# 0xPARC/plonky2-aes

Hardware: AMD Instinct MI355X
Metric: proofs/sec (AES-GCM 1 KiB circuit) (higher is better)
Workload: dtype u64 (Goldilocks field)

## Files before the change

bindings/plonky2-hip/src/ffi.rs:

```rust
#![allow(non_camel_case_types, dead_code)]
use std::os::raw::{c_char, c_int, c_long, c_void};

#[repr(C)] pub struct P2Builder { _private: [u8; 0] }
#[repr(C)] pub struct P2Circuit { _private: [u8; 0] }
#[repr(C)] pub struct P2Assignment { pub targets: *const u64, pub values: *const u64, pub count: usize }
#[repr(C)] #[derive(Default, Clone, Copy)]
pub struct P2CircuitInfo {
    pub degree_bits: u32, pub num_wires: u32, pub num_routed_wires: u32, pub num_constants_cols: u32, pub num_zs_cols: u32,
    pub num_quotient_cols: u32, pub num_luts: u32, pub num_ops: u32, pub num_levels: u32, pub num_slots: u32,
    pub num_virtual_targets: u32, pub num_fri_rounds: u32, pub proof_bytes: u64, pub zero_knowledge: u32, pub num_gate_kinds: u32,
    pub num_public_inputs: u32, pub hasher: u32,
}
#[repr(C)] pub struct P2KernelTime { pub name: [c_char; 48], pub ms: f32, pub count: u32 }
#[repr(C)] #[derive(Default, Clone, Copy, Debug)]
pub struct P2WitnessFault { pub kind: i32, pub op_kind: i32, pub input_index: i64, pub target: u64, pub gate_row: u32, pub computed: u64, pub found: u64 }

pub const P2_OK: c_int = 0;
pub const P2_PROOF_OK: c_int = 0;
pub const P2_VALUE_UNSET: u64 = u64::MAX;
pub const P2_FAULT_KINDS: [&str; 6] = ["NONE", "INPUT_NOT_CANONICAL", "INPUT_CONFLICT", "LOOKUP_MISS", "GENERATOR_CONFLICT", "NOT_SET"];
pub const P2_HASHER_POSEIDON: c_int = 0;
pub const P2_HASHER_KECCAK: c_int = 1;
pub const P2_POINT_WORDS: usize = 10;
pub const P2_SCALAR_LIMBS: usize = 5;
pub const P2_SCALAR_BITS: usize = 320;

#[link(name = "p2aes")]
extern "C" {
    pub fn p2_last_error() -> *const c_char;
    pub fn p2_builder_new() -> *mut P2Builder;
    pub fn p2_builder_new_zk() -> *mut P2Builder;
    pub fn p2_builder_new_config(zero_knowledge: c_int, hasher: c_int) -> *mut P2Builder;
    pub fn p2_builder_set_hasher(a0: *mut P2Builder, hasher: c_int) -> c_int;
    pub fn p2_builder_free(a0: *mut P2Builder);
    pub fn p2_builder_add_virtual_target(a0: *mut P2Builder) -> u64;
    pub fn p2_builder_constant(a0: *mut P2Builder, c: u64) -> u64;
    pub fn p2_builder_zero(a0: *mut P2Builder) -> u64;
    pub fn p2_builder_one(a0: *mut P2Builder) -> u64;
    pub fn p2_builder_arithmetic(a0: *mut P2Builder, c0: u64, c1: u64, m0: u64, m1: u64, addend: u64) -> u64;
    pub fn p2_builder_mul_const_add(a0: *mut P2Builder, c: u64, x: u64, y: u64) -> u64;
    pub fn p2_builder_add(a0: *mut P2Builder, x: u64, y: u64) -> u64;
    pub fn p2_builder_sub(a0: *mut P2Builder, x: u64, y: u64) -> u64;
    pub fn p2_builder_mul(a0: *mut P2Builder, x: u64, y: u64) -> u64;
    pub fn p2_builder_select(a0: *mut P2Builder, b: u64, x: u64, y: u64) -> u64;
    pub fn p2_builder_is_equal(a0: *mut P2Builder, x: u64, y: u64) -> u64;
    pub fn p2_builder_connect(a0: *mut P2Builder, x: u64, y: u64);
    pub fn p2_builder_register_public_input(a0: *mut P2Builder, t: u64) -> c_int;
    pub fn p2_builder_add_lookup_table_from_pairs(a0: *mut P2Builder, pairs: *const u16, n_pairs: usize) -> usize;
    pub fn p2_builder_add_lookup_from_index(a0: *mut P2Builder, looking_in: u64, lut_index: usize) -> u64;
    pub fn p2_builder_num_gates(a0: *const P2Builder) -> usize;
    pub fn p2_builder_build(a0: *mut P2Builder, blob: *mut *mut u8, blob_len: *mut usize) -> c_int;
    pub fn p2_blob_free(blob: *mut u8);
    pub fn p2_aes_sbox_lut(a0: *mut P2Builder) -> usize;
    pub fn p2_aes_byte_xor_lut(a0: *mut P2Builder) -> usize;
    pub fn p2_aes_gf_2_8_mul_lut(a0: *mut P2Builder) -> usize;
    pub fn p2_gcm_u8_unit_right_shift_lut(a0: *mut P2Builder) -> usize;
    pub fn p2_gcm_u8_bitref_lut(a0: *mut P2Builder) -> usize;
    pub fn p2_aes_add_virtual_byte_target(a0: *mut P2Builder, u8_table_idx: usize) -> u64;
    pub fn p2_aes_add_virtual_byte_target_unsafe(a0: *mut P2Builder) -> u64;
    pub fn p2_aes_state_sub_bytes(a0: *mut P2Builder, sbox_lut: usize, s: *const u64, out: *mut u64);
    pub fn p2_aes_state_mix_columns(a0: *mut P2Builder, xor_lut: usize, mul_lut: usize, s: *const u64, out: *mut u64);
    pub fn p2_aes_gf_2_8_mul(a0: *mut P2Builder, mul_lut: usize, x: u64, y: u64) -> u64;
    pub fn p2_aes_gf_2_8_add(a0: *mut P2Builder, xor_lut: usize, x: u64, y: u64) -> u64;
    pub fn p2_aes_key_expansion(a0: *mut P2Builder, nk: c_int, nr: c_int, xor_lut: usize, sbox_lut: usize, key: *const u64, out: *mut u64);
    pub fn p2_aes_encrypt_block(a0: *mut P2Builder, nr: c_int, xor_lut: usize, mul_lut: usize, sbox_lut: usize, state: *const u64, expanded_key: *const u64, out_state: *mut u64);
    pub fn p2_gcm_gctr(a0: *mut P2Builder, nr: c_int, xor_lut: usize, mul_lut: usize, sbox_lut: usize, expanded_key: *const u64, icb: *const u64, x: *const u64, len: usize, y: *mut u64);
    pub fn p2_gcm_right_shift_one(a0: *mut P2Builder, shift_lut: usize, v: *const u64, out: *mut u64);
    pub fn p2_gcm_inc32(a0: *mut P2Builder, block: *const u64, out: *mut u64);
    pub fn p2_gcm_gf_2_128_mul(a0: *mut P2Builder, xor_lut: usize, shift_lut: usize, bitref_lut: usize, x: *const u64, y: *const u64, out: *mut u64);
    pub fn p2_gcm_ghash(a0: *mut P2Builder, xor_lut: usize, shift_lut: usize, bitref_lut: usize, h: *const u64, x: *const u64, len: usize, out: *mut u64) -> c_int;
    pub fn p2_aes_gcm_build(a0: *mut P2Builder, nk: c_int, nr: c_int, L: usize, with_tag: c_int, key: *mut u64, nonce: *mut u64, pt: *mut u64, ct: *mut u64, tag: *mut u64) -> c_int;
    pub fn p2_builder_hash_n_to_m_no_pad(a0: *mut P2Builder, inputs: *const u64, n: usize, outputs: *mut u64, m: usize) -> c_int;
    pub fn p2_poseidon_cipher_build(a0: *mut P2Builder, L: usize, ks: *mut u64, m: *mut u64, nonce: *mut u64, ct: *mut u64) -> c_int;
    pub fn p2_native_hash_n_to_m_no_pad(in: *const u64, n: usize, out: *mut u64, m: usize);
    pub fn p2_native_poseidon_encrypt(ks10: *const u64, msg: *const u64, n_msg: usize, nonce2: *const u64, ct: *mut u64);
    pub fn p2_native_poseidon_decrypt(ks10: *const u64, ct: *const u64, n_ct: usize, nonce2: *const u64, l: usize, msg: *mut u64) -> c_int;
    pub fn p2_ecgfp5_group_order(out: *mut u64);
    pub fn p2_ecgfp5_generator(out: *mut u64);
    pub fn p2_ecgfp5_mul(k: *const u64, p: *const u64, out: *mut u64);
    pub fn p2_ecgfp5_add(p: *const u64, q: *const u64, out: *mut u64);
    pub fn p2_ecgfp5_neg(p: *const u64, out: *mut u64);
    pub fn p2_ecgfp5_is_in_subgroup(p: *const u64) -> c_int;
    pub fn p2_ecgfp5_compress(p: *const u64, w: *mut u64);
    pub fn p2_ecgfp5_decompress(w: *const u64, out: *mut u64) -> c_int;
    pub fn p2_ecgfp5_random_scalar(out: *mut u64) -> c_int;
    pub fn p2_ecgfp5_random_point(out: *mut u64) -> c_int;
    pub fn p2_ecgfp5_encode_binary(limbs: *const u32, out: *mut u64) -> c_int;
    pub fn p2_ecgfp5_random_scalar_seeded(seed: u64, out: *mut u64);
    pub fn p2_ecgfp5_random_point_seeded(seed: u64, out: *mut u64);
    pub fn p2_ecgfp5_encode_binary_seeded(limbs: *const u32, seed: u64, out: *mut u64);
    pub fn p2_ecgfp5_decode_binary(p: *const u64, limbs: *mut u32);
    pub fn p2_elgamal_encrypt(pk: *const u64, nonce: *const u64, msg: *const u64, c0: *mut u64, c1: *mut u64) -> c_int;
    pub fn p2_elgamal_decrypt(sk: *const u64, c0: *const u64, c1: *const u64, msg: *mut u64) -> c_int;
    pub fn p2_hashed_elgamal_encrypt(pk: *const u64, nonce: *const u64, msg: *const u64, c0: *mut u64, ct: *mut u64) -> c_int;
    pub fn p2_hashed_elgamal_decrypt(sk: *const u64, c0: *const u64, ct: *const u64, msg: *mut u64) -> c_int;
    pub fn p2_builder_add_virtual_point_target(a0: *mut P2Builder, out: *mut u64);
    pub fn p2_builder_constant_point(a0: *mut P2Builder, p: *const u64, out: *mut u64);
    pub fn p2_builder_add_virtual_biguint320_target(a0: *mut P2Builder, bits: *mut u64);
    pub fn p2_builder_multiply_point(a0: *mut P2Builder, bits: *const u64, p: *const u64, out: *mut u64) -> c_int;
    pub fn p2_builder_add_point(a0: *mut P2Builder, p: *const u64, q: *const u64, out: *mut u64);
    pub fn p2_builder_public_key(a0: *mut P2Builder, sk_bits: *const u64, pk: *mut u64) -> c_int;
    pub fn p2_builder_elgamal_encrypt(a0: *mut P2Builder, pk: *const u64, nonce_bits: *const u64, msg: *const u64, c0: *mut u64, c1: *mut u64) -> c_int;
    pub fn p2_builder_hashed_elgamal_encrypt(a0: *mut P2Builder, pk: *const u64, nonce_bits: *const u64, msg: *const u64, c0: *mut u64, ct: *mut u64) -> c_int;
    pub fn p2_selftest_host(seed: u64, n_reductions: usize, n_permutations: usize) -> c_int;
    pub fn p2_selftest_device(seed: u64, threads: usize, device: c_int) -> c_int;
    pub fn p2_host_poseidon_known(states: *mut u64, n_perm: usize, kind: c_int, rows: u32, parts: c_int) -> c_int;
    pub fn p2_host_partial_rounds(states: *mut u64, count: usize) -> c_int;
    pub fn p2_host_hash_leaves(data: *const u64, cols: usize, active_cols: usize, num_leaves: usize, digests: *mut u64) -> c_int;
    pub fn p2_native_gf_2_8_mul(a: u8, b: u8) -> u8;
    pub fn p2_native_aes_key_expansion(key: *const u8, nk: c_int, nr: c_int, out: *mut u8);
    pub fn p2_native_aes_encrypt_block(key: *const u8, nk: c_int, nr: c_int, in16: *const u8, out16: *mut u8);
    pub fn p2_native_gf_2_128_mul(x16: *const u8, y16: *const u8, out16: *mut u8);
    pub fn p2_native_ghash(h16: *const u8, x: *const u8, len: usize, out16: *mut u8);
    pub fn p2_native_gctr(key: *const u8, nk: c_int, nr: c_int, icb16: *const u8, x: *const u8, len: usize, y: *mut u8);
    pub fn p2_native_aes_gcm_encrypt(key: *const u8, nk: c_int, nr: c_int, nonce12: *const u8, pt: *const u8, len: usize, ct: *mut u8, tag16: *mut u8);
    pub fn p2_native_keccak_hash_no_pad(in: *const u64, n: usize, out4: *mut u64);
    pub fn p2_native_keccak_two_to_one(l4: *const u64, r4: *const u64, out4: *mut u64);
    pub fn p2_native_keccak256(data: *const u8, len: usize, out32: *mut u8);
    pub fn p2_blob_info(blob: *const u8, len: usize, out: *mut P2CircuitInfo) -> c_int;
    pub fn p2_witness_schedule_check(blob: *const u8, len: usize, fuse: u32, out: *mut u32) -> c_int;
    pub fn p2_verify(blob: *const u8, blob_len: usize, verifier_data: *const u64, verifier_data_len: usize, proof: *const u8, proof_len: usize) -> c_int;
    pub fn p2_proof_compress(blob: *const u8, blob_len: usize, verifier_data: *const u64, verifier_data_len: usize, proof: *const u8, proof_len: usize, out: *mut u8, cap: usize, n_written: *mut usize) -> c_int;
    pub fn p2_proof_decompress(blob: *const u8, blob_len: usize, verifier_data: *const u64, verifier_data_len: usize, cproof: *const u8, cproof_len: usize, out: *mut u8, cap: usize, n_written: *mut usize) -> c_int;
    pub fn p2_verify_compressed(blob: *const u8, blob_len: usize, verifier_data: *const u64, verifier_data_len: usize, cproof: *const u8, cproof_len: usize) -> c_int;
    pub fn p2_proof_public_inputs(blob: *const u8, blob_len: usize, proof: *const u8, proof_len: usize, out: *mut u64, cap: usize, n_written: *mut usize) -> c_int;
    pub fn p2_circuit_load(blob: *const u8, len: usize, device: c_int) -> *mut P2Circuit;
    pub fn p2_circuit_free(a0: *mut P2Circuit);
    pub fn p2_circuit_verifier_data(a0: *const P2Circuit, out: *mut u64, cap: usize, n_written: *mut usize) -> c_int;
    pub fn p2_circuit_chunk_proofs(a0: *mut P2Circuit) -> usize;
    pub fn p2_circuit_set_zk_key(a0: *mut P2Circuit, key: *const u64) -> c_int;
    pub fn p2_circuit_set_zk_seed(a0: *mut P2Circuit, seed: u64) -> c_int;
    pub fn p2_circuit_proof_bytes(a0: *const P2Circuit) -> usize;
    pub fn p2_circuit_num_public_inputs(a0: *const P2Circuit) -> usize;
    pub fn p2_circuit_public_inputs(a0: *const P2Circuit, proof: *const u8, proof_len: usize, out: *mut u64, cap: usize, n_written: *mut usize) -> c_int;
    pub fn p2_prove_batch(a0: *mut P2Circuit, batch: usize, inputs: *const P2Assignment, proofs: *mut u8, status: *mut c_int) -> c_int;
    pub fn p2_prove_batch_multi(handles: *const *mut P2Circuit, n_handles: usize, batch: usize, inputs: *const P2Assignment, proofs: *mut u8, status: *mut c_int) -> c_int;
    pub fn p2_prove_batch_device(a0: *mut P2Circuit, batch: usize, targets: *const u64, n_targets: usize, d_values: *const u64, d_proofs: *mut u8, d_status: *mut c_int, stream: *mut c_void) -> c_int;
    pub fn p2_circuit_synchronize(a0: *mut P2Circuit) -> c_int;
    pub fn p2_prove_batch_outputs_device(a0: *mut P2Circuit, batch: usize, targets: *const u64, n_targets: usize, d_values: *const u64, out_targets: *const u64, n_out: usize, d_out: *mut u64, d_proofs: *mut u8, d_status: *mut c_int, stream: *mut c_void) -> c_int;
    pub fn p2_prove_batch_outputs(a0: *mut P2Circuit, batch: usize, inputs: *const P2Assignment, out_targets: *const u64, n_out: usize, out_values: *mut u64, proofs: *mut u8, status: *mut c_int) -> c_int;
    pub fn p2_witness_batch_device(a0: *mut P2Circuit, batch: usize, targets: *const u64, n_targets: usize, d_values: *const u64, out_targets: *const u64, n_out: usize, d_out: *mut u64, d_status: *mut c_int, stream: *mut c_void) -> c_int;
    pub fn p2_witness_batch(a0: *mut P2Circuit, batch: usize, inputs: *const P2Assignment, out_targets: *const u64, n_out: usize, out_values: *mut u64, status: *mut c_int) -> c_int;
    pub fn p2_witness_explain(a0: *mut P2Circuit, input: *const P2Assignment, status: *mut c_int, out: *mut c_void) -> c_int;
    pub fn p2_host_witness(blob: *const u8, len: usize, input: *const P2Assignment, out_targets: *const u64, n_out: usize, out_values: *mut u64, status: *mut c_int, fault: *mut c_void) -> c_int;
    pub fn p2_verify_batch(a0: *mut P2Circuit, batch: usize, proofs: *const u8, verifier_data: *const u64, vd_len: usize, status: *mut c_int) -> c_int;
    pub fn p2_verify_batch_device(a0: *mut P2Circuit, batch: usize, d_proofs: *const u8, verifier_data: *const u64, vd_len: usize, d_status: *mut c_int, stream: *mut c_void) -> c_int;
    pub fn p2_compress_batch(a0: *mut P2Circuit, batch: usize, proofs: *const u8, verifier_data: *const u64, vd_len: usize, out: *mut u8, lengths: *mut u32, status: *mut c_int) -> c_int;
    pub fn p2_decompress_batch(a0: *mut P2Circuit, batch: usize, cproofs: *const u8, lengths: *const u32, verifier_data: *const u64, vd_len: usize, out: *mut u8, status: *mut c_int) -> c_int;
    pub fn p2_verify_compressed_batch(a0: *mut P2Circuit, batch: usize, cproofs: *const u8, lengths: *const u32, verifier_data: *const u64, vd_len: usize, status: *mut c_int) -> c_int;
    pub fn p2_compress_batch_device(a0: *mut P2Circuit, batch: usize, d_proofs: *const u8, verifier_data: *const u64, vd_len: usize, d_out: *mut u8, d_lengths: *mut u32, d_status: *mut c_int, stream: *mut c_void) -> c_int;
    pub fn p2_decompress_batch_device(a0: *mut P2Circuit, batch: usize, d_cproofs: *const u8, d_lengths: *const u32, verifier_data: *const u64, vd_len: usize, d_out: *mut u8, d_status: *mut c_int, stream: *mut c_void) -> c_int;
    pub fn p2_verify_compressed_batch_device(a0: *mut P2Circuit, batch: usize, d_cproofs: *const u8, d_lengths: *const u32, verifier_data: *const u64, vd_len: usize, d_status: *mut c_int, stream: *mut c_void) -> c_int;
    pub fn p2_circuit_set_option(a0: *mut P2Circuit, name: *const c_char, value: c_long) -> c_int;
    pub fn p2_circuit_set_timing(a0: *mut P2Circuit, enable: c_int) -> c_int;
    pub fn p2_circuit_get_timing(a0: *mut P2Circuit, out: *mut P2KernelTime, cap: usize) -> usize;
    pub fn p2_gpu_device_count() -> c_int;
    pub fn p2_gpu_poseidon(states: *mut u64, n_perm: usize, device: c_int) -> c_int;
    pub fn p2_gpu_lde(coeffs: *const u64, cols: usize, degree_bits: c_int, rate_bits: c_int, lde: *mut u64, device: c_int) -> c_int;
    pub fn p2_gpu_intt(values: *const u64, cols: usize, degree_bits: c_int, coeffs: *mut u64, device: c_int) -> c_int;
    pub fn p2_gpu_merkle_cap(cols_major: *const u64, cols: usize, num_leaves: usize, cap_height: c_int, cap: *mut u64, device: c_int) -> c_int;
    pub fn p2_gpu_merkle_cap_hasher(cols_major: *const u64, cols: usize, num_leaves: usize, cap_height: c_int, hasher: c_int, cap: *mut u64, device: c_int) -> c_int;
    pub fn p2_gpu_hash_leaves(data: *const u64, cols: usize, active_cols: usize, num_leaves: usize, batch: usize, digests: *mut u64, device: c_int) -> c_int;
    pub fn p2_gpu_partial_rounds(states: *mut u64, count: usize, device: c_int) -> c_int;
    pub fn p2_gpu_merkle_level(child: *const u64, num_parents: usize, batch: usize, parent: *mut u64, device: c_int) -> c_int;
    pub fn p2_gpu_hash_fri_leaves(vals: *const u64, len: usize, arity: c_int, batch: usize, digests: *mut u64, device: c_int) -> c_int;
    pub fn p2_circuit_debug_read(a0: *mut P2Circuit, name: *const c_char, index: usize, out: *mut u64, cap: usize, n_written: *mut usize) -> c_int;
}
```

include/p2aes.h:

```cpp
#ifndef P2AES_H
#define P2AES_H
#include <stddef.h>
#include <stdint.h>

#ifdef __cplusplus
extern "C" {
#endif

enum {
    P2_OK = 0,
    P2_ERR_INVALID = 1,
    P2_ERR_NO_DEVICE = 2,
    P2_ERR_HIP = 3,
    P2_ERR_VERIFY = 4
};
enum {
    P2_PROOF_OK = 0,
    P2_PROOF_WITNESS_CONFLICT = 1,
    P2_PROOF_MISSING_INPUT = 2,
    P2_PROOF_ZETA_IN_SUBGROUP = 3,
    P2_PROOF_POW_NOT_FOUND = 4
};
enum {
    P2_VERIFY_OK = 0,
// ... 26 lines not shown
p2_target p2_builder_arithmetic(p2_builder*, uint64_t c0, uint64_t c1, p2_target m0, p2_target m1, p2_target addend);
p2_target p2_builder_mul_const_add(p2_builder*, uint64_t c, p2_target x, p2_target y);
p2_target p2_builder_add(p2_builder*, p2_target x, p2_target y);
p2_target p2_builder_sub(p2_builder*, p2_target x, p2_target y);
p2_target p2_builder_mul(p2_builder*, p2_target x, p2_target y);
p2_target p2_builder_select(p2_builder*, p2_target b, p2_target x, p2_target y);
p2_target p2_builder_is_equal(p2_builder*, p2_target x, p2_target y);
void p2_builder_connect(p2_builder*, p2_target x, p2_target y);
int p2_builder_register_public_input(p2_builder*, p2_target t);
size_t p2_builder_add_lookup_table_from_pairs(p2_builder*, const uint16_t* pairs, size_t n_pairs);
p2_target p2_builder_add_lookup_from_index(p2_builder*, p2_target looking_in, size_t lut_index);
size_t p2_builder_num_gates(const p2_builder*);
int p2_builder_build(p2_builder*, uint8_t** blob, size_t* blob_len);
void p2_blob_free(uint8_t* blob);

size_t p2_aes_sbox_lut(p2_builder*);
size_t p2_aes_byte_xor_lut(p2_builder*);
size_t p2_aes_gf_2_8_mul_lut(p2_builder*);
size_t p2_gcm_u8_unit_right_shift_lut(p2_builder*);
size_t p2_gcm_u8_bitref_lut(p2_builder*);
p2_target p2_aes_add_virtual_byte_target(p2_builder*, size_t u8_table_idx);
p2_target p2_aes_add_virtual_byte_target_unsafe(p2_builder*);
void p2_aes_state_sub_bytes(p2_builder*, size_t sbox_lut, const p2_target* s, p2_target* out);
void p2_aes_state_mix_columns(p2_builder*, size_t xor_lut, size_t mul_lut, const p2_target* s, p2_target* out);
p2_target p2_aes_gf_2_8_mul(p2_builder*, size_t mul_lut, p2_target x, p2_target y);
p2_target p2_aes_gf_2_8_add(p2_builder*, size_t xor_lut, p2_target x, p2_target y);
void p2_aes_key_expansion(p2_builder*, int nk, int nr, size_t xor_lut, size_t sbox_lut, const p2_target* key, p2_target* out);
void p2_aes_encrypt_block(p2_builder*, int nr, size_t xor_lut, size_t mul_lut, size_t sbox_lut, const p2_target* state,
                          const p2_target* expanded_key, p2_target* out_state);
void p2_gcm_gctr(p2_builder*, int nr, size_t xor_lut, size_t mul_lut, size_t sbox_lut, const p2_target* expanded_key,
                 const p2_target* icb, const p2_target* x, size_t len, p2_target* y);
void p2_gcm_right_shift_one(p2_builder*, size_t shift_lut, const p2_target* v, p2_target* out);
void p2_gcm_inc32(p2_builder*, const p2_target* block, p2_target* out);
void p2_gcm_gf_2_128_mul(p2_builder*, size_t xor_lut, size_t shift_lut, size_t bitref_lut, const p2_target* x,
                         const p2_target* y, p2_target* out);
int p2_gcm_ghash(p2_builder*, size_t xor_lut, size_t shift_lut, size_t bitref_lut, const p2_target* h, const p2_target* x,
                 size_t len, p2_target* out);
int p2_aes_gcm_build(p2_builder*, int nk, int nr, size_t L, int with_tag, p2_target* key, p2_target* nonce, p2_target* pt,
                     p2_target* ct, p2_target* tag);

int p2_builder_hash_n_to_m_no_pad(p2_builder*, const p2_target* inputs, size_t n, p2_target* outputs, size_t m);
int p2_poseidon_cipher_build(p2_builder*, size_t L, p2_target* ks, p2_target* m, p2_target* nonce, p2_target* ct);
void p2_native_hash_n_to_m_no_pad(const uint64_t* in, size_t n, uint64_t* out, size_t m);
void p2_native_poseidon_encrypt(const uint64_t* ks10, const uint64_t* msg, size_t n_msg, const uint64_t* nonce2, uint64_t* ct);
int p2_native_poseidon_decrypt(const uint64_t* ks10, const uint64_t* ct, size_t n_ct, const uint64_t* nonce2, size_t l, uint64_t* msg);

#define P2_POINT_WORDS 10
#define P2_SCALAR_LIMBS 5
#define P2_SCALAR_BITS 320
void p2_ecgfp5_group_order(uint64_t out[5]);
void p2_ecgfp5_generator(uint64_t out[10]);
void p2_ecgfp5_mul(const uint64_t k[5], const uint64_t p[10], uint64_t out[10]);
void p2_ecgfp5_add(const uint64_t p[10], const uint64_t q[10], uint64_t out[10]);
void p2_ecgfp5_neg(const uint64_t p[10], uint64_t out[10]);
int p2_ecgfp5_is_in_subgroup(const uint64_t p[10]);
void p2_ecgfp5_compress(const uint64_t p[10], uint64_t w[5]);
int p2_ecgfp5_decompress(const uint64_t w[5], uint64_t out[10]);
int p2_ecgfp5_random_scalar(uint64_t out[5]);
int p2_ecgfp5_random_point(uint64_t out[10]);
int p2_ecgfp5_encode_binary(const uint32_t limbs[5], uint64_t out[10]);
void p2_ecgfp5_random_scalar_seeded(uint64_t seed, uint64_t out[5]);
void p2_ecgfp5_random_point_seeded(uint64_t seed, uint64_t out[10]);
void p2_ecgfp5_encode_binary_seeded(const uint32_t limbs[5], uint64_t seed, uint64_t out[10]);
void p2_ecgfp5_decode_binary(const uint64_t p[10], uint32_t limbs[5]);
int p2_elgamal_encrypt(const uint64_t pk[10], const uint64_t nonce[5], const uint64_t msg[10], uint64_t c0[10], uint64_t c1[10]);
int p2_elgamal_decrypt(const uint64_t sk[5], const uint64_t c0[10], const uint64_t c1[10], uint64_t msg[10]);
int p2_hashed_elgamal_encrypt(const uint64_t pk[10], const uint64_t nonce[5], const uint64_t msg[5], uint64_t c0[10], uint64_t ct[5]);
int p2_hashed_elgamal_decrypt(const uint64_t sk[5], const uint64_t c0[10], const uint64_t ct[5], uint64_t msg[5]);
void p2_builder_add_virtual_point_target(p2_builder*, p2_target out[10]);
void p2_builder_constant_point(p2_builder*, const uint64_t p[10], p2_target out[10]);
void p2_builder_add_virtual_biguint320_target(p2_builder*, p2_target bits[320]);
int p2_builder_multiply_point(p2_builder*, const p2_target bits[320], const p2_target p[10], p2_target out[10]);
void p2_builder_add_point(p2_builder*, const p2_target p[10], const p2_target q[10], p2_target out[10]);
int p2_builder_public_key(p2_builder*, const p2_target sk_bits[320], p2_target pk[10]);
int p2_builder_elgamal_encrypt(p2_builder*, const p2_target pk[10], const p2_target nonce_bits[320], const p2_target msg[10],
                               p2_target c0[10], p2_target c1[10]);
int p2_builder_hashed_elgamal_encrypt(p2_builder*, const p2_target pk[10], const p2_target nonce_bits[320], const p2_target msg[5],
                                      p2_target c0[10], p2_target ct[5]);

int p2_selftest_host(uint64_t seed, size_t n_reductions, size_t n_permutations);
int p2_selftest_device(uint64_t seed, size_t threads, int device);
int p2_host_poseidon_known(uint64_t* states, size_t n_perm, int kind, uint32_t rows, int parts);
int p2_host_partial_rounds(uint64_t* states, size_t count);
int p2_host_hash_leaves(const uint64_t* data, size_t cols, size_t active_cols, size_t num_leaves, uint64_t* digests);

uint8_t p2_native_gf_2_8_mul(uint8_t a, uint8_t b);
void p2_native_aes_key_expansion(const uint8_t* key, int nk, int nr, uint8_t* out );
void p2_native_aes_encrypt_block(const uint8_t* key, int nk, int nr, const uint8_t* in16, uint8_t* out16);
void p2_native_gf_2_128_mul(const uint8_t* x16, const uint8_t* y16, uint8_t* out16);
void p2_native_ghash(const uint8_t* h16, const uint8_t* x, size_t len, uint8_t* out16);
void p2_native_gctr(const uint8_t* key, int nk, int nr, const uint8_t* icb16, const uint8_t* x, size_t len, uint8_t* y);
void p2_native_aes_gcm_encrypt(const uint8_t* key, int nk, int nr, const uint8_t* nonce12, const uint8_t* pt, size_t len,
                               uint8_t* ct, uint8_t* tag16);

void p2_native_keccak_hash_no_pad(const uint64_t* in, size_t n, uint64_t out4[4]);
void p2_native_keccak_two_to_one(const uint64_t l4[4], const uint64_t r4[4], uint64_t out4[4]);
void p2_native_keccak256(const uint8_t* data, size_t len, uint8_t out32[32]);

typedef struct {
    uint32_t degree_bits, num_wires, num_routed_wires, num_constants_cols, num_zs_cols, num_quotient_cols, num_luts,
        num_ops, num_levels, num_slots, num_virtual_targets, num_fri_rounds;
    uint64_t proof_bytes;
    uint32_t zero_knowledge, num_gate_kinds;
    uint32_t num_public_inputs;
    uint32_t hasher;
} p2_circuit_info;
int p2_blob_info(const uint8_t* blob, size_t len, p2_circuit_info* out);
int p2_witness_schedule_check(const uint8_t* blob, size_t len, uint32_t fuse, uint32_t out[4]);
int p2_verify(const uint8_t* blob, size_t blob_len, const uint64_t* verifier_data, size_t verifier_data_len,
              const uint8_t* proof, size_t proof_len);
int p2_proof_compress(const uint8_t* blob, size_t blob_len, const uint64_t* verifier_data, size_t verifier_data_len, const uint8_t* proof,
                      size_t proof_len, uint8_t* out, size_t cap, size_t* n_written);
int p2_proof_decompress(const uint8_t* blob, size_t blob_len, const uint64_t* verifier_data, size_t verifier_data_len, const uint8_t* cproof,
                        size_t cproof_len, uint8_t* out, size_t cap, size_t* n_written);
int p2_verify_compressed(const uint8_t* blob, size_t blob_len, const uint64_t* verifier_data, size_t verifier_data_len,
                         const uint8_t* cproof, size_t cproof_len);
int p2_proof_public_inputs(const uint8_t* blob, size_t blob_len, const uint8_t* proof, size_t proof_len, uint64_t* out, size_t cap,
                           size_t* n_written);

typedef struct p2_circuit p2_circuit;
p2_circuit* p2_circuit_load(const uint8_t* blob, size_t len, int device);
void p2_circuit_free(p2_circuit*);
int p2_circuit_verifier_data(const p2_circuit*, uint64_t* out, size_t cap, size_t* n_written);
size_t p2_circuit_chunk_proofs(p2_circuit*);
int p2_circuit_set_zk_key(p2_circuit*, const uint64_t key[4]);
int p2_circuit_set_zk_seed(p2_circuit*, uint64_t seed);
size_t p2_circuit_proof_bytes(const p2_circuit*);
size_t p2_circuit_num_public_inputs(const p2_circuit*);
int p2_circuit_public_inputs(const p2_circuit*, const uint8_t* proof, size_t proof_len, uint64_t* out, size_t cap, size_t* n_written);
typedef struct {
    const p2_target* targets;
    const uint64_t* values;
    size_t count;
} p2_assignment;
int p2_prove_batch(p2_circuit*, size_t batch, const p2_assignment* inputs, uint8_t* proofs, int* status);
int p2_prove_batch_multi(p2_circuit* const* handles, size_t n_handles, size_t batch, const p2_assignment* inputs,
                         uint8_t* proofs, int* status);
int p2_prove_batch_device(p2_circuit*, size_t batch, const p2_target* targets, size_t n_targets, const uint64_t* d_values,
                          uint8_t* d_proofs, int* d_status, void* stream);
int p2_circuit_synchronize(p2_circuit*);

#define P2_VALUE_UNSET UINT64_MAX
int p2_prove_batch_outputs_device(p2_circuit*, size_t batch, const p2_target* targets, size_t n_targets, const uint64_t* d_values,
                                  const p2_target* out_targets, size_t n_out, uint64_t* d_out, uint8_t* d_proofs, int* d_status, void* stream);
int p2_prove_batch_outputs(p2_circuit*, size_t batch, const p2_assignment* inputs, const p2_target* out_targets, size_t n_out,
                           uint64_t* out_values, uint8_t* proofs, int* status);
int p2_witness_batch_device(p2_circuit*, size_t batch, const p2_target* targets, size_t n_targets, const uint64_t* d_values,
                            const p2_target* out_targets, size_t n_out, uint64_t* d_out, int* d_status, void* stream);
int p2_witness_batch(p2_circuit*, size_t batch, const p2_assignment* inputs, const p2_target* out_targets, size_t n_out,
                     uint64_t* out_values, int* status);
typedef struct {
    int32_t kind;
    int32_t op_kind;
    int64_t input_index;
    p2_target target;
    uint32_t gate_row;
    uint64_t computed, found;
} p2_witness_fault;
enum {
    P2_FAULT_NONE = 0,
    P2_FAULT_INPUT_NOT_CANONICAL = 1,
    P2_FAULT_INPUT_CONFLICT = 2,
    P2_FAULT_LOOKUP_MISS = 3,
    P2_FAULT_GENERATOR_CONFLICT = 4,
    P2_FAULT_NOT_SET = 5
};
int p2_witness_explain(p2_circuit*, const p2_assignment* input, int* status, void* out);
int p2_host_witness(const uint8_t* blob, size_t len, const p2_assignment* input, const p2_target* out_targets, size_t n_out,
                    uint64_t* out_values, int* status, void* fault);

int p2_verify_batch(p2_circuit*, size_t batch, const uint8_t* proofs, const uint64_t* verifier_data, size_t vd_len, int* status);
int p2_verify_batch_device(p2_circuit*, size_t batch, const uint8_t* d_proofs, const uint64_t* verifier_data, size_t vd_len,
                           int* d_status, void* stream);
int p2_compress_batch(p2_circuit*, size_t batch, const uint8_t* proofs, const uint64_t* verifier_data, size_t vd_len, uint8_t* out,
                      uint32_t* lengths, int* status);
int p2_decompress_batch(p2_circuit*, size_t batch, const uint8_t* cproofs, const uint32_t* lengths, const uint64_t* verifier_data,
                        size_t vd_len, uint8_t* out, int* status);
int p2_verify_compressed_batch(p2_circuit*, size_t batch, const uint8_t* cproofs, const uint32_t* lengths, const uint64_t* verifier_data,
                               size_t vd_len, int* status);
int p2_compress_batch_device(p2_circuit*, size_t batch, const uint8_t* d_proofs, const uint64_t* verifier_data, size_t vd_len,
                             uint8_t* d_out, uint32_t* d_lengths, int* d_status, void* stream);
int p2_decompress_batch_device(p2_circuit*, size_t batch, const uint8_t* d_cproofs, const uint32_t* d_lengths,
                               const uint64_t* verifier_data, size_t vd_len, uint8_t* d_out, int* d_status, void* stream);
int p2_verify_compressed_batch_device(p2_circuit*, size_t batch, const uint8_t* d_cproofs, const uint32_t* d_lengths,
                                      const uint64_t* verifier_data, size_t vd_len, int* d_status, void* stream);
int p2_circuit_set_option(p2_circuit*, const char* name, long value);
typedef struct {
    char name[48];
    float ms;
    uint32_t count;
} p2_kernel_time;
int p2_circuit_set_timing(p2_circuit*, int enable);
size_t p2_circuit_get_timing(p2_circuit*, p2_kernel_time* out, size_t cap);

int p2_gpu_device_count(void);
int p2_gpu_poseidon(uint64_t* states, size_t n_perm, int device);
int p2_gpu_lde(const uint64_t* coeffs, size_t cols, int degree_bits, int rate_bits, uint64_t* lde, int device);
int p2_gpu_intt(const uint64_t* values, size_t cols, int degree_bits, uint64_t* coeffs, int device);
int p2_gpu_merkle_cap(const uint64_t* cols_major, size_t cols, size_t num_leaves, int cap_height, uint64_t* cap, int device);
int p2_gpu_merkle_cap_hasher(const uint64_t* cols_major, size_t cols, size_t num_leaves, int cap_height, int hasher, uint64_t* cap, int device);
int p2_gpu_hash_leaves(const uint64_t* data, size_t cols, size_t active_cols, size_t num_leaves, size_t batch, uint64_t* digests, int device);
int p2_gpu_partial_rounds(uint64_t* states, size_t count, int device);
int p2_gpu_merkle_level(const uint64_t* child, size_t num_parents, size_t batch, uint64_t* parent, int device);
int p2_gpu_hash_fri_leaves(const uint64_t* vals, size_t len, int arity, size_t batch, uint64_t* digests, int device);
int p2_circuit_debug_read(p2_circuit*, const char* name, size_t index, uint64_t* out, size_t cap, size_t* n_written);

#ifdef __cplusplus
}
#endif
#endif
```

plonky2-aes_amd/api.py:

```python
import ctypes as C
import os
import struct

P = 0xFFFFFFFF00000001


class P2Error(RuntimeError):
    pass


class ProveError(P2Error):

    def __init__(self, status):
        self.status = status
        super().__init__({1: "witness conflict or lookup input not in table", 2: "a generator never ran (missing input)",
                          3: "opening point is in the subgroup",
                          4: "no proof-of-work witness found"}.get(status, "prove failed (%d)" % status))


VERIFY_OK, VERIFY_SHAPE, VERIFY_NON_CANONICAL, VERIFY_POW, VERIFY_ZETA_IN_SUBGROUP, VERIFY_VANISHING = 0, 1, 2, 3, 4, 5
VERIFY_MERKLE_INITIAL, VERIFY_FRI_FOLD, VERIFY_MERKLE_FRI, VERIFY_FINAL_POLY = 6, 7, 8, 9
VERIFY_REASONS = {
    "": VERIFY_OK,
    "proof truncated": VERIFY_SHAPE,
# ... 137 lines not shown
        "p2_proof_public_inputs": (C.c_int, [C.c_char_p, sz, C.c_char_p, sz, u64p, sz, C.POINTER(sz)]),
        "p2_builder_add_lookup_table_from_pairs": (sz, [vp, u16p, sz]),
        "p2_builder_add_lookup_from_index": (u64, [vp, u64, sz]),
        "p2_builder_num_gates": (sz, [vp]),
        "p2_builder_build": (C.c_int, [vp, C.POINTER(u8p), C.POINTER(sz)]), "p2_blob_free": (None, [u8p]),
        "p2_aes_sbox_lut": (sz, [vp]), "p2_aes_byte_xor_lut": (sz, [vp]), "p2_aes_gf_2_8_mul_lut": (sz, [vp]),
        "p2_gcm_u8_unit_right_shift_lut": (sz, [vp]), "p2_gcm_u8_bitref_lut": (sz, [vp]),
        "p2_aes_add_virtual_byte_target": (u64, [vp, sz]), "p2_aes_add_virtual_byte_target_unsafe": (u64, [vp]),
        "p2_aes_state_sub_bytes": (None, [vp, sz, u64p, u64p]),
        "p2_aes_state_mix_columns": (None, [vp, sz, sz, u64p, u64p]),
        "p2_aes_gf_2_8_mul": (u64, [vp, sz, u64, u64]), "p2_aes_gf_2_8_add": (u64, [vp, sz, u64, u64]),
        "p2_aes_key_expansion": (None, [vp, C.c_int, C.c_int, sz, sz, u64p, u64p]),
        "p2_aes_encrypt_block": (None, [vp, C.c_int, sz, sz, sz, u64p, u64p, u64p]),
        "p2_gcm_gctr": (None, [vp, C.c_int, sz, sz, sz, u64p, u64p, u64p, sz, u64p]),
        "p2_gcm_right_shift_one": (None, [vp, sz, u64p, u64p]), "p2_gcm_inc32": (None, [vp, u64p, u64p]),
        "p2_gcm_gf_2_128_mul": (None, [vp, sz, sz, sz, u64p, u64p, u64p]),
        "p2_gcm_ghash": (C.c_int, [vp, sz, sz, sz, u64p, u64p, sz, u64p]),
        "p2_aes_gcm_build": (C.c_int, [vp, C.c_int, C.c_int, sz, C.c_int, u64p, u64p, u64p, u64p, u64p]),
        "p2_builder_hash_n_to_m_no_pad": (C.c_int, [vp, u64p, sz, u64p, sz]),
        "p2_poseidon_cipher_build": (C.c_int, [vp, sz, u64p, u64p, u64p, u64p]),
        "p2_native_hash_n_to_m_no_pad": (None, [u64p, sz, u64p, sz]),
        "p2_native_poseidon_encrypt": (None, [u64p, u64p, sz, u64p, u64p]),
        "p2_native_poseidon_decrypt": (C.c_int, [u64p, u64p, sz, u64p, sz, u64p]),
        "p2_ecgfp5_group_order": (None, [u64p]), "p2_ecgfp5_generator": (None, [u64p]),
        "p2_ecgfp5_mul": (None, [u64p, u64p, u64p]), "p2_ecgfp5_add": (None, [u64p, u64p, u64p]), "p2_ecgfp5_neg": (None, [u64p, u64p]),
        "p2_ecgfp5_is_in_subgroup": (C.c_int, [u64p]),
        "p2_ecgfp5_compress": (None, [u64p, u64p]), "p2_ecgfp5_decompress": (C.c_int, [u64p, u64p]),
        "p2_ecgfp5_random_scalar": (C.c_int, [u64p]), "p2_ecgfp5_random_point": (C.c_int, [u64p]),
        "p2_ecgfp5_encode_binary": (C.c_int, [u32p, u64p]),
        "p2_ecgfp5_random_scalar_seeded": (None, [u64, u64p]), "p2_ecgfp5_random_point_seeded": (None, [u64, u64p]),
        "p2_ecgfp5_encode_binary_seeded": (None, [u32p, u64, u64p]), "p2_ecgfp5_decode_binary": (None, [u64p, u32p]),
        "p2_elgamal_encrypt": (C.c_int, [u64p, u64p, u64p, u64p, u64p]), "p2_elgamal_decrypt": (C.c_int, [u64p, u64p, u64p, u64p]),
        "p2_hashed_elgamal_encrypt": (C.c_int, [u64p, u64p, u64p, u64p, u64p]),
        "p2_hashed_elgamal_decrypt": (C.c_int, [u64p, u64p, u64p, u64p]),
        "p2_builder_add_virtual_point_target": (None, [vp, u64p]), "p2_builder_constant_point": (None, [vp, u64p, u64p]),
        "p2_builder_add_virtual_biguint320_target": (None, [vp, u64p]),
        "p2_builder_multiply_point": (C.c_int, [vp, u64p, u64p, u64p]), "p2_builder_add_point": (None, [vp, u64p, u64p, u64p]),
        "p2_builder_public_key": (C.c_int, [vp, u64p, u64p]),
        "p2_builder_elgamal_encrypt": (C.c_int, [vp, u64p, u64p, u64p, u64p, u64p]),
        "p2_builder_hashed_elgamal_encrypt": (C.c_int, [vp, u64p, u64p, u64p, u64p, u64p]),
        "p2_selftest_host": (C.c_int, [u64, sz, sz]), "p2_selftest_device": (C.c_int, [u64, sz, C.c_int]),
        "p2_native_gf_2_8_mul": (C.c_uint8, [C.c_uint8, C.c_uint8]),
        "p2_native_aes_key_expansion": (None, [C.c_char_p, C.c_int, C.c_int, C.c_char_p]),
        "p2_native_aes_encrypt_block": (None, [C.c_char_p, C.c_int, C.c_int, C.c_char_p, C.c_char_p]),
        "p2_native_gf_2_128_mul": (None, [C.c_char_p, C.c_char_p, C.c_char_p]),
        "p2_native_ghash": (None, [C.c_char_p, C.c_char_p, sz, C.c_char_p]),
        "p2_native_gctr": (None, [C.c_char_p, C.c_int, C.c_int, C.c_char_p, C.c_char_p, sz, C.c_char_p]),
        "p2_native_aes_gcm_encrypt": (None, [C.c_char_p, C.c_int, C.c_int, C.c_char_p, C.c_char_p, sz, C.c_char_p, C.c_char_p]),
        "p2_blob_info": (C.c_int, [C.c_char_p, sz, C.POINTER(_Info)]),
        "p2_witness_schedule_check": (C.c_int, [C.c_char_p, sz, C.c_uint32, u32p]),
        "p2_verify": (C.c_int, [C.c_char_p, sz, u64p, sz, C.c_char_p, sz]),
        "p2_proof_compress": (C.c_int, [C.c_char_p, sz, u64p, sz, C.c_char_p, sz, C.c_char_p, sz, C.POINTER(sz)]),
        "p2_proof_decompress": (C.c_int, [C.c_char_p, sz, u64p, sz, C.c_char_p, sz, C.c_char_p, sz, C.POINTER(sz)]),
        "p2_verify_compressed": (C.c_int, [C.c_char_p, sz, u64p, sz, C.c_char_p, sz]),
        "p2_circuit_load": (vp, [C.c_char_p, sz, C.c_int]), "p2_circuit_free": (None, [vp]),
        "p2_circuit_verifier_data": (C.c_int, [vp, u64p, sz, C.POINTER(sz)]),
        "p2_circuit_proof_bytes": (sz, [vp]),
        "p2_circuit_num_public_inputs": (sz, [vp]),
        "p2_circuit_public_inputs": (C.c_int, [vp, C.c_char_p, sz, u64p, sz, C.POINTER(sz)]),
        "p2_circuit_chunk_proofs": (sz, [vp]),
        "p2_prove_batch": (C.c_int, [vp, sz, C.POINTER(_Assignment), C.c_char_p, C.POINTER(C.c_int)]),
        "p2_prove_batch_device": (C.c_int, [vp, sz, u64p, sz, vp, vp, vp, vp]),
        "p2_circuit_synchronize": (C.c_int, [vp]),
        "p2_prove_batch_outputs": (C.c_int, [vp, sz, C.POINTER(_Assignment), u64p, sz, u64p, C.c_char_p, C.POINTER(C.c_int)]),
        "p2_prove_batch_outputs_device": (C.c_int, [vp, sz, u64p, sz, vp, u64p, sz, vp, vp, vp, vp]),
        "p2_witness_batch": (C.c_int, [vp, sz, C.POINTER(_Assignment), u64p, sz, u64p, C.POINTER(C.c_int)]),
        "p2_witness_batch_device": (C.c_int, [vp, sz, u64p, sz, vp, u64p, sz, vp, vp, vp]),
        "p2_witness_explain": (C.c_int, [vp, C.POINTER(_Assignment), C.POINTER(C.c_int), vp]),
        "p2_host_witness": (C.c_int, [C.c_char_p, sz, C.POINTER(_Assignment), u64p, sz, u64p, C.POINTER(C.c_int), vp]),
        "p2_verify_batch": (C.c_int, [vp, sz, C.c_char_p, u64p, sz, C.POINTER(C.c_int)]),
        "p2_verify_batch_device": (C.c_int, [vp, sz, vp, u64p, sz, vp, vp]),
        "p2_compress_batch": (C.c_int, [vp, sz, C.c_char_p, u64p, sz, C.c_char_p, u32p, C.POINTER(C.c_int)]),
        "p2_compress_batch_device": (C.c_int, [vp, sz, vp, u64p, sz, vp, vp, vp, vp]),
        "p2_decompress_batch": (C.c_int, [vp, sz, C.c_char_p, u32p, u64p, sz, C.c_char_p, C.POINTER(C.c_int)]),
        "p2_decompress_batch_device": (C.c_int, [vp, sz, vp, vp, u64p, sz, vp, vp, vp]),
        "p2_verify_compressed_batch": (C.c_int, [vp, sz, C.c_char_p, u32p, u64p, sz, C.POINTER(C.c_int)]),
        "p2_verify_compressed_batch_device": (C.c_int, [vp, sz, vp, vp, u64p, sz, vp, vp]),
        "p2_circuit_set_timing": (C.c_int, [vp, C.c_int]),
        "p2_circuit_get_timing": (sz, [vp, C.POINTER(_KernelTime), sz]),
        "p2_gpu_device_count": (C.c_int, []),
        "p2_gpu_poseidon": (C.c_int, [u64p, sz, C.c_int]),
        "p2_host_partial_rounds": (C.c_int, [u64p, sz]),
        "p2_gpu_partial_rounds": (C.c_int, [u64p, sz, C.c_int]),
        "p2_gpu_lde": (C.c_int, [u64p, sz, C.c_int, C.c_int, u64p, C.c_int]),
        "p2_gpu_intt": (C.c_int, [u64p, sz, C.c_int, u64p, C.c_int]),
        "p2_gpu_merkle_cap": (C.c_int, [u64p, sz, sz, C.c_int, u64p, C.c_int]),
        "p2_circuit_debug_read": (C.c_int, [vp, C.c_char_p, sz, u64p, sz, C.POINTER(sz)]),
    }
    missing = []
    for name, (res, args) in sig.items():
        try:
            f = getattr(L, name)
        except AttributeError:
            missing.append(name)
            continue
        f.restype, f.argtypes = res, args
    L._p2_missing = missing
    L._p2_signatures = sig
    _lib = L
    return L


def _err():
    return lib().p2_last_error().decode()


def _arr(vals):
    return (u64 * len(vals))(*vals)


class CircuitBuilder:
    def __init__(self, zero_knowledge=False, hasher="poseidon"):
        if hasher not in HASHERS:
            raise P2Error("unknown hasher %r (known: %s)" % (hasher, ", ".join(sorted(HASHERS))))
        if hasher == "poseidon":
            self._h = lib().p2_builder_new_zk() if zero_knowledge else lib().p2_builder_new()
        else:
            self._h = lib().p2_builder_new_config(1 if zero_knowledge else 0, HASHERS[hasher])
        if not self._h:
            raise P2Error(_err())

    def __del__(self):
        if getattr(self, "_h", None):
            lib().p2_builder_free(self._h)
            self._h = None

    def add_virtual_target(self): return lib().p2_builder_add_virtual_target(self._h)
    def add_virtual_target_arr(self, n): return [self.add_virtual_target() for _ in range(n)]
    def constant(self, c): return lib().p2_builder_constant(self._h, c % P)
    def zero(self): return lib().p2_builder_zero(self._h)
    def one(self): return lib().p2_builder_one(self._h)
    def arithmetic(self, c0, c1, m0, m1, addend): return lib().p2_builder_arithmetic(self._h, c0 % P, c1 % P, m0, m1, addend)
    def mul_const_add(self, c, x, y): return lib().p2_builder_mul_const_add(self._h, c % P, x, y)
    def add(self, x, y): return lib().p2_builder_add(self._h, x, y)
    def sub(self, x, y): return lib().p2_builder_sub(self._h, x, y)
    def mul(self, x, y): return lib().p2_builder_mul(self._h, x, y)
    def select(self, b, x, y): return lib().p2_builder_select(self._h, b, x, y)
    def is_equal(self, x, y): return lib().p2_builder_is_equal(self._h, x, y)
    def connect(self, x, y): lib().p2_builder_connect(self._h, x, y)

    def register_public_input(self, t):
        if lib().p2_builder_register_public_input(self._h, t):
            raise P2Error(_err())

    def register_public_inputs(self, ts):
        for t in ts:
            self.register_public_input(t)

    def add_lookup_table_from_pairs(self, pairs):
        flat = (C.c_uint16 * (2 * len(pairs)))(*[v for p in pairs for v in p])
        return lib().p2_builder_add_lookup_table_from_pairs(self._h, flat, len(pairs))

    def add_lookup_from_index(self, looking_in, lut_index):
        t = lib().p2_builder_add_lookup_from_index(self._h, looking_in, lut_index)
        if t == 0xFFFFFFFFFFFFFFFF:
            raise P2Error(_err())
        return t

    def num_gates(self): return lib().p2_builder_num_gates(self._h)

    def sbox_lut(self): return lib().p2_aes_sbox_lut(self._h)
    def byte_xor_lut(self): return lib().p2_aes_byte_xor_lut(self._h)
    def gf_2_8_mul_lut(self): return lib().p2_aes_gf_2_8_mul_lut(self._h)
    def u8_unit_right_shift_lut(self): return lib().p2_gcm_u8_unit_right_shift_lut(self._h)
    def u8_bitref_lut(self): return lib().p2_gcm_u8_bitref_lut(self._h)
    def add_virtual_byte_target(self, u8_table_idx): return lib().p2_aes_add_virtual_byte_target(self._h, u8_table_idx)
# ... 722 lines not shown
```

plonky2-aes_amd/csrc/capi_host.cpp:

```cpp
#include <stdlib.h>

#include "../../include/p2aes.h"
#include "aes_gadgets.h"
#include "capi_common.h"
#include "compress.h"
#include "ecgfp5.h"
#include "poseidon_cipher.h"
#include "poseidon_fast.h"
#include "verifier.h"
#include "witness_check.h"
#include "witness_schedule.h"

using namespace p2;

namespace p2 {
thread_local std::string g_last_error;
}

struct p2_builder {
    CircuitBuilder b;
};


template <class F>
// ... 409 lines not shown
                               p2_target c1[10]) {
    try {
        ecgfp5::PointTarget a, c;
        ecgfp5::elgamal_encrypt_target(b->b, ptt_at(pk), bits_at(nonce_bits), ptt_at(msg), &a, &c);
        ptt_put(a, c0);
        ptt_put(c, c1);
        return P2_OK;
    } catch (std::exception& e) {
        return set_error(e.what()), P2_ERR_INVALID;
    }
}
int p2_builder_hashed_elgamal_encrypt(p2_builder* b, const p2_target pk[10], const p2_target nonce_bits[320], const p2_target msg[5],
                                      p2_target c0[10], p2_target ct[5]) {
    try {
        ecgfp5::PointTarget a;
        ecgfp5::hashed_elgamal_encrypt_target(b->b, ptt_at(pk), bits_at(nonce_bits), msg, &a, ct);
        ptt_put(a, c0);
        return P2_OK;
    } catch (std::exception& e) {
        return set_error(e.what()), P2_ERR_INVALID;
    }
}

int p2_selftest_host(uint64_t seed, size_t n_reductions, size_t n_permutations) {
    u64 x = seed | 1;
    auto rnd = [&]() {
        x ^= x << 13;
        x ^= x >> 7;
        x ^= x << 17;
        return x;
    };
    size_t bad = 0;
    for (size_t i = 0; i < n_reductions; i++) {
        u64 hi = rnd(), lo = rnd();
        switch (i & 15) {
            case 0: hi &= gl::EPS; break;
            case 1: lo &= gl::EPS; break;
            case 2: hi |= ~gl::EPS; break;
            case 3: lo |= ~gl::EPS; break;
            case 4: hi = 0; break;
            case 5: lo = 0; break;
            case 6: hi = ~0ull; lo = ~0ull - (x & 3); break;
            case 7: hi &= ~gl::EPS; lo &= gl::EPS; break;
            default: break;
        }
        unsigned __int128 v = ((unsigned __int128)hi << 64) | lo;
        u64 want = (u64)(v % gl::P);
        if (glf::canon(glf::red128(hi, lo)) != want) bad++;
        if (gl::reduce128(hi, lo) != want) bad++;
        glf::Acc a;
        a.init();
        a.fma(hi, lo);
        a.fma(lo, lo);
        unsigned __int128 w = ((unsigned __int128)hi * lo) % gl::P + ((unsigned __int128)lo * lo) % gl::P;
        if (glf::canon(a.reduce()) != (u64)(w % gl::P)) bad++;
    }
    for (size_t i = 0; i < n_permutations; i++) {
        u64 s0[12], s1[12];
        for (int k = 0; k < 12; k++) s0[k] = s1[k] = (i & 3) == 3 ? rnd() : rnd() % gl::P;
        for (int k = 0; k < 12; k++) s0[k] %= gl::P;
        gl::poseidon(s0);
        glf::poseidon(s1);
        for (int k = 0; k < 12; k++) bad += s0[k] != s1[k];
    }
    return (int)std::min<size_t>(bad, 0x7FFFFFFF);
}

int p2_host_poseidon_known(uint64_t* states, size_t n_perm, int kind, uint32_t rows, int parts) {
    if (kind < 0 || kind > (int)glf::FR_ZERO_RATE || rows == 0 || rows > glf::ROWS_ALL) return set_error("kind must be 0..2 and rows a mask of words 0..11"), P2_ERR_INVALID;
    for (size_t i = 0; i < n_perm; i++) {
        u64* s = states + 12 * i;
        if (parts) {
            glf::first_round_any(s, (u32)kind);
            glf::middle(s);
            glf::last_round_any(s, rows);
        } else {
            glf::permute_known_any(s, (u32)kind, rows);
        }
    }
    return P2_OK;
}
int p2_host_partial_rounds(uint64_t* states, size_t count) {
    for (size_t i = 0; i < count; i++) glf::partial_block(states + 12 * i);
    return P2_OK;
}
int p2_host_hash_leaves(const uint64_t* data, size_t cols, size_t active_cols, size_t num_leaves, uint64_t* digests) {
    if (cols == 0 || cols > (1u << 20)) return set_error("cols out of range"), P2_ERR_INVALID;
    for (size_t leaf = 0; leaf < num_leaves; leaf++) {
        u64 st[12] = {0};
        u64* out = digests + 4 * leaf;
        if (cols <= 4) {
            for (size_t c = 0; c < 4; c++) out[c] = (c < cols && c < active_cols) ? data[c * num_leaves + leaf] : 0;
            continue;
        }
        for (size_t c0 = 0; c0 < cols; c0 += 8) {
            for (size_t k = 0; k < 8 && c0 + k < cols; k++) st[k] = c0 + k < active_cols ? data[(c0 + k) * num_leaves + leaf] : 0;
            glf::sponge_permute(st, (int)c0, (int)cols, (int)std::min(active_cols, cols));
        }
        for (int i = 0; i < 4; i++) out[i] = st[i];
    }
    return P2_OK;
}

uint8_t p2_native_gf_2_8_mul(uint8_t a, uint8_t b) { return aes::gf_2_8_mul(a, b); }
void p2_native_aes_key_expansion(const uint8_t* key, int nk, int nr, uint8_t* out) {
    (void)guarded([&] {
        auto w = aes::key_expansion(nk, nr, key);
        for (size_t i = 0; i < w.size(); i++) memcpy(out + 4 * i, w[i].data(), 4);
    });
}
void p2_native_aes_encrypt_block(const uint8_t* key, int nk, int nr, const uint8_t* in, uint8_t* out) {
    (void)guarded([&] {
        auto w = aes::key_expansion(nk, nr, key);
        auto s = aes::flatten_state(aes::encrypt_block(nr, in, w));
        memcpy(out, s.data(), 16);
    });
}
void p2_native_gf_2_128_mul(const uint8_t* x, const uint8_t* y, uint8_t* out) {
    (void)guarded([&] {
        auto r = aes::gf_2_128_mul(x, y);
        memcpy(out, r.data(), 16);
    });
}
void p2_native_ghash(const uint8_t* h, const uint8_t* x, size_t len, uint8_t* out) {
    (void)guarded([&] {
        auto r = aes::ghash(h, x, len);
        memcpy(out, r.data(), 16);
    });
}
void p2_native_gctr(const uint8_t* key, int nk, int nr, const uint8_t* icb, const uint8_t* x, size_t len, uint8_t* y) {
    (void)guarded([&] {
        auto w = aes::key_expansion(nk, nr, key);
        auto r = aes::gctr(nr, w, icb, x, len);
        if (len) memcpy(y, r.data(), len);
    });
}
void p2_native_aes_gcm_encrypt(const uint8_t* key, int nk, int nr, const uint8_t* nonce, const uint8_t* pt, size_t len, uint8_t* ct, uint8_t* tag) { (void)guarded([&] {    aes::gcm_encrypt(nk, nr, key, nonce, pt, len, ct, tag);}); }

int p2_blob_info(const uint8_t* blob, size_t len, p2_circuit_info* out) {
    try {
        Circuit c = deserialize(blob, len);
        fill_info(c, out);
        return P2_OK;
    } catch (std::exception& e) {
        return set_error(e.what()), P2_ERR_INVALID;
    }
}
int p2_witness_schedule_check(const uint8_t* blob, size_t len, uint32_t fuse, uint32_t out[4]) {
    try {
        Circuit c = deserialize(blob, len);
        WitnessSchedule s = schedule_witness(c, fuse);
        const size_t M = c.ops.size(), n = (size_t)1 << c.degree_bits;
        const u32 R = c.cfg.num_routed_wires;
        auto same = [](const Op& x, const Op& y) { return x.kind == y.kind && x.out == y.out && x.a == y.a && x.b == y.b && x.c == y.c && x.aux == y.aux && x.k0 == y.k0 && x.k1 == y.k1; };
        auto slots_of = [&](const Op& o, u32* d, int& first_out) {
            int nd = 0;
            if (o.kind == OP_ARITH) d[nd++] = o.a, d[nd++] = o.b, d[nd++] = o.c;
            else if (o.kind == OP_LOOKUP) d[nd++] = o.a;
            else if (o.kind == OP_EQ || o.kind == OP_EQINV) d[nd++] = o.a, d[nd++] = o.b;
            else if (o.kind == OP_POSEIDON) {
                for (u32 k = 0; k < 12; k++) d[nd++] = (u32)c.wire_slot[(size_t)(PG_IN + k) * n + o.a];
                d[nd++] = (u32)c.wire_slot[(size_t)PG_SWAP * n + o.a];
            }
            first_out = nd;
            if (o.kind == OP_POSEIDON) {
                for (u32 col = PG_OUT; col < R; col++)
// ... 229 lines not shown
```

plonky2-aes_amd/csrc/kernels.h:

```cpp
#pragma once
#include <hip/hip_runtime.h>

#include "circuit.h"
#include "witness_schedule.h"
#include "gl.h"
#include "poseidon_fast.h"
#include "poseidon_gate.h"
#include "zk_prf.h"

namespace p2k {
using gl::E2;
using gl::u32;
using gl::u64;

static const u64 UNSET = ~0ull;

#ifndef P2_HASH_WAVES_PER_EU
#define P2_HASH_WAVES_PER_EU 5
#endif
#define P2_HASH_WAVES __attribute__((amdgpu_waves_per_eu(P2_HASH_WAVES_PER_EU, P2_HASH_WAVES_PER_EU)))

__global__ __launch_bounds__(256) P2_HASH_WAVES void k_hash_leaves(const u64* __restrict__ data, int cols, int active_cols, size_t col_stride,
                                                      size_t batch_stride, size_t num_leaves, u64* __restrict__ digests,
                                                      size_t dig_batch_stride) {
// ... 39 lines not shown
        }
        glf::sponge_permute(st, e0, width, width);
    }
    u64* out = digests + (size_t)blockIdx.y * dig_batch_stride + leaf * 4;
#pragma unroll
    for (int i = 0; i < 4; i++) out[i] = st[i];
}

__global__ __launch_bounds__(256) P2_HASH_WAVES void k_merkle_level(const u64* __restrict__ child, u64* __restrict__ parent, size_t num_parents,
                                                       size_t batch_stride) {
    if ((size_t)blockIdx.x * blockDim.x + threadIdx.x >= num_parents) return;
    u64 st[12];
    {
        const u64* c = child + (size_t)blockIdx.y * batch_stride + 8 * ((size_t)blockIdx.x * blockDim.x + threadIdx.x);
#pragma unroll
        for (int k = 0; k < 8; k++) st[k] = c[k];
    }
#pragma unroll
    for (int k = 8; k < 12; k++) st[k] = 0;
    glf::two_to_one_permute(st);
    u64* o = parent + (size_t)blockIdx.y * batch_stride + 4 * ((size_t)blockIdx.x * blockDim.x + threadIdx.x);
#pragma unroll
    for (int k = 0; k < 4; k++) o[k] = st[k];
}

__global__ __launch_bounds__(256) P2_HASH_WAVES void k_merkle_top(u64* __restrict__ dig, size_t batch_stride, u32 bits, u32 first_level, u32 num_levels) {
    u64* base = dig + (size_t)blockIdx.y * batch_stride;
    u32 P = ((1u << bits) >> (first_level + 1)) / gridDim.x;
    for (u32 k = 0, l = first_level; k < num_levels; k++, l++, P >>= 1) {
        if (threadIdx.x < P) {
            const size_t off_c = 4 * (((size_t)2 << bits) - ((size_t)2 << (bits - l))), off_p = 4 * (((size_t)2 << bits) - ((size_t)2 << (bits - l - 1)));
            const size_t idx = (size_t)blockIdx.x * P + threadIdx.x;
            u64 st[12];
            {
                const u64* c = base + off_c + 8 * idx;
#pragma unroll
                for (int q = 0; q < 8; q++) st[q] = c[q];
            }
#pragma unroll
            for (int q = 8; q < 12; q++) st[q] = 0;
            glf::two_to_one_permute(st);
            u64* o = base + off_p + 4 * idx;
#pragma unroll
            for (int q = 0; q < 4; q++) o[q] = st[q];
        }
        __syncthreads();
    }
}
__global__ __launch_bounds__(256) void k_merkle_top_coop(u64* __restrict__ dig, size_t batch_stride, u32 bits, u32 first_level, u32 num_levels) {
    u64* base = dig + (size_t)blockIdx.y * batch_stride;
    u32 P = ((1u << bits) >> (first_level + 1)) / gridDim.x;
    const u32 g = threadIdx.x >> 4, i = threadIdx.x & 15;
    for (u32 k = 0, l = first_level; k < num_levels; k++, l++, P >>= 1) {
        const size_t off_c = 4 * (((size_t)2 << bits) - ((size_t)2 << (bits - l))), off_p = 4 * (((size_t)2 << bits) - ((size_t)2 << (bits - l - 1)));
        for (u32 first = 0; first < P; first += blockDim.x >> 4) {
            if (first + ((threadIdx.x >> 6) << 2) < P) {
                const u32 idx = first + g;
                const bool live = idx < P;
                const size_t node = (size_t)blockIdx.x * P + (live ? idx : 0);
                u64 w = (live && i < 8) ? base[off_c + 8 * node + i] : 0;
                w = glf::poseidon_coop(w, i);
                if (live && i < 4) base[off_p + 4 * node + i] = w;
            }
        }
        __syncthreads();
    }
}

__global__ void k_poseidon_states(u64* states, size_t n) {
    size_t i = (size_t)blockIdx.x * blockDim.x + threadIdx.x;
    if (i >= n) return;
    u64 st[12];
    for (int k = 0; k < 12; k++) st[k] = states[12 * i + k];
    glf::poseidon(st);
    for (int k = 0; k < 12; k++) states[12 * i + k] = st[k];
}

__global__ __launch_bounds__(256) P2_HASH_WAVES void k_partial_rounds(u64* states, size_t n) {
    size_t i = (size_t)blockIdx.x * blockDim.x + threadIdx.x;
    if (i >= n) return;
    u64 st[12];
    for (int k = 0; k < 12; k++) st[k] = states[12 * i + k];
    glf::partial_block(st);
    for (int k = 0; k < 12; k++) states[12 * i + k] = st[k];
}

struct NttArgs {
    const u64* in;
    u64* out;
    const u64* tw;
    const u64* pre;
    const u64* pre_tw;
    const u64* post;
    u64 post_scalar;
    size_t in_col_stride, out_col_stride, in_batch_stride, out_batch_stride;
    int logn, log_nmax, cosets;
    int bitrev_in, bitrev_out;
    int in_coset_blocks;
    u32 block_of_coset[8];
};

__global__ __launch_bounds__(1024) void k_ntt_lds(NttArgs a) {
    extern __shared__ __align__(16) u64 lds[];
    const int logn = a.logn;
    const u32 n = 1u << logn;
    const u32 col = blockIdx.x / a.cosets, coset = blockIdx.x % a.cosets;
    const u32 blk = a.block_of_coset[coset];
    const u64* in = a.in + (size_t)blockIdx.y * a.in_batch_stride + (size_t)col * a.in_col_stride + (a.in_coset_blocks ? (size_t)blk * n : 0);
    u64* out = a.out + (size_t)blockIdx.y * a.out_batch_stride + (size_t)col * a.out_col_stride + (size_t)blk * n;
    const u64* pre = a.pre ? a.pre + (size_t)coset * n : nullptr;
    const u64* post = a.post ? a.post + (size_t)coset * n : nullptr;
    for (u32 i = threadIdx.x; i < n; i += blockDim.x) {
        u64 v = in[i];
        u32 dst = a.bitrev_in ? (__brev(i) >> (32 - logn)) : i;
        if (pre) v = gl::mul_nb(v, pre[dst]);
        lds[dst] = v;
    }
    __syncthreads();
    const int tw_shift = a.log_nmax - logn;
    int s = logn - 1;
    if (logn & 1) {
        const u32 h = 1u << s;
        for (u32 t = threadIdx.x; t < (n >> 1); t += blockDim.x) {
            u32 pos = t & (h - 1);
            u32 i = ((t >> s) << (s + 1)) | pos;
            u64 x = lds[i], y = lds[i + h];
            u64 w = a.tw[(size_t)(pos << (logn - 1 - s)) << tw_shift];
            lds[i] = gl::add(x, y);
            lds[i + h] = gl::mul_nb(gl::sub(x, y), w);
        }
        __syncthreads();
        s--;
    }
    for (; s >= 1; s -= 2) {
        const u32 h = 1u << s, q = h >> 1;
        for (u32 t = threadIdx.x; t < (n >> 2); t += blockDim.x) {
            u32 pos = t & (q - 1);
            u32 i = ((t >> (s - 1)) << (s + 1)) | pos;
            u64 a0 = lds[i], a1 = lds[i + q], a2 = lds[i + h], a3 = lds[i + h + q];
            u64 w0 = a.tw[(size_t)(pos << (logn - 1 - s)) << tw_shift];
            u64 w1 = a.tw[(size_t)((pos + q) << (logn - 1 - s)) << tw_shift];
            u64 b0 = gl::add(a0, a2), b2 = gl::mul_nb(gl::sub(a0, a2), w0);
            u64 b1 = gl::add(a1, a3), b3 = gl::mul_nb(gl::sub(a1, a3), w1);
            u64 w2 = a.tw[(size_t)(pos << (logn - s)) << tw_shift];
            lds[i] = gl::add(b0, b1);
            lds[i + q] = gl::mul_nb(gl::sub(b0, b1), w2);
            lds[i + h] = gl::add(b2, b3);
            lds[i + h + q] = gl::mul_nb(gl::sub(b2, b3), w2);
        }
        __syncthreads();
    }
    for (u32 i = threadIdx.x; i < n; i += blockDim.x) {
        u32 src = a.bitrev_out ? (__brev(i) >> (32 - logn)) : i;
        u64 v = lds[src];
        if (post)
            v = gl::mul_nb(v, post[i]);
        else if (a.post_scalar != 1)
            v = gl::mul_nb(v, a.post_scalar);
        out[i] = v;
    }
}

__device__ __forceinline__ u32 ntt_pad(u32 i) { return i + (i >> 4); }
struct NttLdsWalk {
    u32 a0, step;
    __device__ __forceinline__ NttLdsWalk(u32 base, u32 stride) : a0(8 * ntt_pad(base)), step(stride >= 16 ? 8 * (stride + (stride >> 4)) : 8 * stride) {}
// ... 854 lines not shown
            for (int i = 0; i < 4; i++) dl[i] = c.challenge();
        if (writer) {
            for (int i = 0; i < 2; i++) ch[CH_BETAS + i] = bg[i];
            for (int i = 0; i < 2; i++) ch[CH_GAMMAS + i] = bg[2 + i];
            if (a.aux) {
                for (int i = 0; i < 4; i++) ch[CH_DELTAS + i] = bg[i];
                for (int i = 0; i < 4; i++) ch[CH_DELTAS + 4 + i] = dl[i];
            }
        }
    } else if (a.stage == 1) {
        const u64 a0 = c.challenge(), a1 = c.challenge();
        if (writer) ch[CH_ALPHAS] = a0, ch[CH_ALPHAS + 1] = a1;
    } else if (a.stage == 2) {
        const u64 z0 = c.challenge(), z1 = c.challenge();
        if (writer) {
            ch[CH_ZETA] = z0;
            ch[CH_ZETA + 1] = z1;
            E2 zp = gl::exp_pow2(gl::e2(z0, z1), (int)a.aux);
            if (zp.a == 1 && zp.b == 0) atomicMax(&a.status[p], 3);
        }
    } else if (a.stage == 3) {
        const u64 f0 = c.challenge(), f1 = c.challenge();
        if (writer) ch[CH_FRI_ALPHA] = f0, ch[CH_FRI_ALPHA + 1] = f1;
    } else if (a.stage == 4) {
        const u64 b0 = c.challenge(), b1 = c.challenge();
        if (writer) ch[CH_FRI_BETAS + 2 * a.aux] = b0, ch[CH_FRI_BETAS + 2 * a.aux + 1] = b1;
    }
    if (real) c.store(a.st[p]);
}

__global__ __launch_bounds__(64) void k_pi_hash(const u64* __restrict__ values, u32 num_slots, const u32* __restrict__ pi_slots, u32 k, u32 batch,
                                                u64* __restrict__ pi_hash, uint8_t* __restrict__ proofs, size_t proof_bytes, size_t trailer_off) {
    const u32 t = blockIdx.x * blockDim.x + threadIdx.x;
    const bool real = (t >> 4) < batch;
    const u32 p = real ? (t >> 4) : batch - 1;
    const u32 i = t & 15;
    const u64* v = values + (size_t)p * num_slots;
    uint8_t* tr = proofs + (size_t)p * proof_bytes + trailer_off;
    if (real) {
        for (u32 j = i; j < k; j += 16) {
            const u64 x = v[pi_slots[j]];
#pragma unroll
            for (int b = 0; b < 8; b++) tr[8 + 8 * (size_t)j + b] = (uint8_t)(x >> (8 * b));
        }
        if (i == 0)
#pragma unroll
            for (int b = 0; b < 8; b++) tr[b] = (uint8_t)((u64)k >> (8 * b));
    }
    u64 w = 0;
    for (u32 off = 0; off < k; off += 8) {
        if (i < 8 && off + i < k) w = v[pi_slots[off + i]];
        w = glf::poseidon_coop(w, i);
    }
    if (real && i < 4) pi_hash[(size_t)p * 4 + i] = w;
}

static const u32 POW_PHASE_BLOCKS[3] = {1u << 8, 3u << 8, 7u << 10};
static const u32 POW_PHASE_SLOTS[3] = {0, 64, 8};
__global__ __launch_bounds__(256) void k_pow(const ChalState* st, u64* chal, int pow_bits, unsigned long long* best , u32 block0,
                                             const u32* list , const u32* count) {
    __shared__ u64 sh[12];
    __shared__ u32 sh_pos;
    __shared__ unsigned long long sh_cur;
    const u64 block_start = ((u64)block0 + blockIdx.y) * blockDim.x;
    const u32 n_items = list ? *count : gridDim.x;
    for (u32 item = blockIdx.x; item < n_items; item += gridDim.x) {
        const u32 p = list ? list[item] : item;
        __syncthreads();
        if (threadIdx.x == 0) sh_cur = atomicMin(&best[p], ~0ull);
        __syncthreads();
        if (sh_cur < block_start) continue;
        if (threadIdx.x < 12) {
            const ChalState* s = st + p;
            u32 i = threadIdx.x;
            sh[i] = (i < s->in_len) ? s->in[i] : s->state[i];
            if (i == 0) sh_pos = s->in_len;
        }
        __syncthreads();
        const u64 cand = block_start + threadIdx.x;
        const u32 pos = sh_pos;
        u64 r[12];
#pragma unroll
        for (int i = 0; i < 12; i++) r[i] = ((u32)i == pos) ? cand : sh[i];
        glf::poseidon(r);
        if ((r[7] >> (64 - pow_bits)) == 0) atomicMin(&best[p], (unsigned long long)cand);
    }
}
__global__ void k_pow_compact(const unsigned long long* best, u32 batch, u32* list, u32* count) {
    __shared__ u32 n;
    if (threadIdx.x == 0) n = 0;
    __syncthreads();
    for (u32 p = threadIdx.x; p < batch; p += blockDim.x)
        if (best[p] == ~0ull) list[atomicAdd(&n, 1u)] = p;
    __syncthreads();
    if (threadIdx.x == 0) *count = n;
}
__global__ void k_pow_finish(u64* chal, const unsigned long long* best, u32 batch, int* status) {
    u32 p = blockIdx.x * blockDim.x + threadIdx.x;
    if (p >= batch) return;
    chal[(size_t)p * CH_WORDS + CH_POW] = best[p];
    if (best[p] == ~0ull) atomicMax(&status[p], 4);
}

template <bool MUL>
__device__ __forceinline__ u64 block_scan_inclusive(u64 v, u64* lds) {
    const u32 t = threadIdx.x;
    lds[t] = v;
    __syncthreads();
    for (u32 off = 1; off < blockDim.x; off <<= 1) {
        u64 x = lds[t];
        u64 y = t >= off ? lds[t - off] : (MUL ? 1 : 0);
        __syncthreads();
        lds[t] = MUL ? gl::mul(x, y) : gl::add(x, y);
        __syncthreads();
    }
    return lds[t];
}

static const u32 PERM_MAX_CHUNKS = 12;
__global__ __launch_bounds__(256) void k_perm_chunks(const u64* __restrict__ wires, size_t wires_batch_stride, const u64* __restrict__ sigmas,
                                                     const u64* __restrict__ k_is, const u64* __restrict__ subgroup, const u64* __restrict__ chal,
                                                     u64* __restrict__ q, size_t q_batch_stride, u32 n, u32 num_routed, u32 chunk_size, u32 num_chunks,
                                                     u32 num_challenges) {
    const u32 row = blockIdx.x * blockDim.x + threadIdx.x;
    if (row >= n) return;
    const u64* cw = chal + (size_t)blockIdx.y * CH_WORDS;
    const u64* w = wires + (size_t)blockIdx.y * wires_batch_stride + row;
    const u64* sg = sigmas + row;
    const bool two = num_challenges > 1;
    const u64 b0 = cw[CH_BETAS], g0 = cw[CH_GAMMAS], b1 = two ? cw[CH_BETAS + 1] : 0, g1 = two ? cw[CH_GAMMAS + 1] : 0;
    const u64 x = subgroup[row], bx0 = gl::mul(b0, x), bx1 = gl::mul(b1, x);
    u64 num[2 * PERM_MAX_CHUNKS], den[2 * PERM_MAX_CHUNKS], pre[2 * PERM_MAX_CHUNKS];
#pragma unroll
    for (u32 c = 0; c < PERM_MAX_CHUNKS; c++) {
        u64 n0 = 1, d0 = 1, n1 = 1, d1 = 1;
        if (c < num_chunks) {
            const u32 j1 = min(num_routed, (c + 1) * chunk_size);
            for (u32 j = c * chunk_size; j < j1; j++) {
                const u64 wv = w[(size_t)j * n], s = sg[(size_t)j * n], kj = k_is[j];
                n0 = gl::mul(n0, gl::add(gl::add(wv, gl::mul(bx0, kj)), g0));
                d0 = gl::mul(d0, gl::add(gl::add(wv, gl::mul(b0, s)), g0));
                if (two) {
                    n1 = gl::mul(n1, gl::add(gl::add(wv, gl::mul(bx1, kj)), g1));
                    d1 = gl::mul(d1, gl::add(gl::add(wv, gl::mul(b1, s)), g1));
                }
            }
        }
        num[c] = n0;
        den[c] = d0;
        num[PERM_MAX_CHUNKS + c] = n1;
        den[PERM_MAX_CHUNKS + c] = d1;
    }
    u64 run = 1;
#pragma unroll
    for (u32 k = 0; k < 2 * PERM_MAX_CHUNKS; k++) {
        pre[k] = run;
        run = gl::mul(run, den[k]);
    }
    u64 inv = gl::inv(run);
#pragma unroll
    for (u32 kk = 2 * PERM_MAX_CHUNKS; kk-- > 0;) {
        const u64 dinv = gl::mul(inv, pre[kk]);
        inv = gl::mul(inv, den[kk]);
        const u32 ch = kk / PERM_MAX_CHUNKS, c = kk % PERM_MAX_CHUNKS;
        if (c < num_chunks && ch < num_challenges)
            q[(size_t)blockIdx.y * q_batch_stride + ((size_t)ch * num_chunks + c) * n + row] = gl::mul(num[kk], dinv);
    }
// ... 170 lines not shown
```

plonky2-aes_amd/csrc/poseidon_fast.h:

```cpp
#pragma once
#include "gl.h"

namespace glf {
using gl::u32;
using gl::u64;

#if defined(__HIP_DEVICE_COMPILE__)
#define P2F_DECL __device__ __constant__ static
#else
#define P2F_DECL static
#endif
#include "poseidon_fast.inc"
P2F_DECL const unsigned long long PF_ZERO12[12] = {0, 0, 0, 0, 0, 0, 0, 0, 0, 0, 0, 0};

GL_HD void mul128(u64 a, u64 b, u64& hi, u64& lo) {
#if defined(__HIP_DEVICE_COMPILE__)
    u32 a0 = (u32)a, a1 = (u32)(a >> 32), b0 = (u32)b, b1 = (u32)(b >> 32);
    u64 p00 = (u64)a0 * b0;
    u64 mid = (u64)a0 * b1 + (p00 >> 32);
    u64 mid2 = (u64)a1 * b0 + (u32)mid;
    lo = (mid2 << 32) | (u32)p00;
    hi = (u64)a1 * b1 + (mid >> 32) + (mid2 >> 32);
#else
    unsigned __int128 m = (unsigned __int128)a * b;
// ... 61 lines not shown
            "v_addc_co_u32_e64 %[co], %[s2], 0, %[co], %[s2]\n\t"
            "v_addc_co_u32_e64 %[ce2], %[s3], 0, %[ce2], %[s3]\n\t"
            "v_addc_co_u32_e64 %[co], %[s4], 0, %[co], %[s4]"
            : [e01] "+v"(e01), [o01] "+v"(o01), [e23] "+v"(e23), [ce0] "+v"(ce0), [co] "+v"(co), [ce2] "+v"(ce2), [s1] "=&s"(s1), [s2] "=&s"(s2),
              [s3] "=&s"(s3), [s4] "=&s"(s4)
            : [a0] "v"(a0), [a1] "v"(a1), [b0] "v"(b0), [b1] "v"(b1));
#else
        u64 p, t;
        p = (u64)a0 * b0; t = e01 + p; ce0 += t < p; e01 = t;
        p = (u64)a0 * b1; t = o01 + p; co += t < p; o01 = t;
        p = (u64)a1 * b1; t = e23 + p; ce2 += t < p; e23 = t;
        p = (u64)a1 * b0; t = o01 + p; co += t < p; o01 = t;
#endif
    }
    GL_HD void fma_k(u64 k, u64 b) {
#if defined(__HIP_DEVICE_COMPILE__)
        const u32 a0 = (u32)k, a1 = (u32)(k >> 32), b0 = (u32)b, b1 = (u32)(b >> 32);
        unsigned long long s1, s2, s3, s4;
        asm("v_mad_u64_u32 %[e01], %[s1], %[a0], %[b0], %[e01]\n\t"
            "v_mad_u64_u32 %[o01], %[s2], %[a0], %[b1], %[o01]\n\t"
            "v_mad_u64_u32 %[e23], %[s3], %[a1], %[b1], %[e23]\n\t"
            "v_addc_co_u32_e64 %[ce0], %[s1], 0, %[ce0], %[s1]\n\t"
            "v_mad_u64_u32 %[o01], %[s4], %[a1], %[b0], %[o01]\n\t"
            "v_addc_co_u32_e64 %[co], %[s2], 0, %[co], %[s2]\n\t"
            "v_addc_co_u32_e64 %[ce2], %[s3], 0, %[ce2], %[s3]\n\t"
            "v_addc_co_u32_e64 %[co], %[s4], 0, %[co], %[s4]"
            : [e01] "+v"(e01), [o01] "+v"(o01), [e23] "+v"(e23), [ce0] "+v"(ce0), [co] "+v"(co), [ce2] "+v"(ce2), [s1] "=&s"(s1), [s2] "=&s"(s2),
              [s3] "=&s"(s3), [s4] "=&s"(s4)
            : [a0] "s"(a0), [a1] "s"(a1), [b0] "v"(b0), [b1] "v"(b1));
#else
        fma(k, b);
#endif
    }
    GL_HD void fma_small(u32 a0, u64 b) {
        u32 b0 = (u32)b, b1 = (u32)(b >> 32);
#if defined(__HIP_DEVICE_COMPILE__)
        unsigned long long s1, s2;
        asm("v_mad_u64_u32 %[e01], %[s1], %[a0], %[b0], %[e01]\n\t"
            "v_mad_u64_u32 %[o01], %[s2], %[a0], %[b1], %[o01]\n\t"
            "s_nop 0\n\t"
            "v_addc_co_u32_e64 %[ce0], %[s1], 0, %[ce0], %[s1]\n\t"
            "v_addc_co_u32_e64 %[co], %[s2], 0, %[co], %[s2]"
            : [e01] "+v"(e01), [o01] "+v"(o01), [ce0] "+v"(ce0), [co] "+v"(co), [s1] "=&s"(s1), [s2] "=&s"(s2)
            : [a0] "v"(a0), [b0] "v"(b0), [b1] "v"(b1));
#else
        u64 p, t;
        p = (u64)a0 * b0; t = e01 + p; ce0 += t < p; e01 = t;
        p = (u64)a0 * b1; t = o01 + p; co += t < p; o01 = t;
#endif
    }
    GL_HD u64 reduce() const {
        u32 k1, k2, k2b, k3, k3b, b, b2;
        const u32 L0 = (u32)e01;
        const u32 L1 = __builtin_addc((u32)(e01 >> 32), (u32)o01, 0u, &k1);
        u32 L2 = __builtin_addc((u32)(o01 >> 32), (u32)e23, k1, &k2);
        L2 = __builtin_addc(L2, ce0, 0u, &k2b);
        u32 L3 = __builtin_addc((u32)(e23 >> 32), co, k2, &k3);
        L3 = __builtin_addc(L3, 0u, k2b, &k3b);
        const u32 L4 = ce2 + k3 + k3b;
        const u64 r = red128(((u64)L3 << 32) | L2, ((u64)L1 << 32) | L0);
        const u32 h1 = __builtin_subc((u32)(r >> 32), L4, 0u, &b);
        u32 lo = __builtin_subc((u32)r, 0u - b, 0u, &b2);
        u32 hi = h1 - b2;
#if defined(__HIP_DEVICE_COMPILE__)
        asm("" : "+v"(lo), "+v"(hi));
#endif
        return ((u64)hi << 32) | lo;
    }
};

GL_HD u64 add_wrap(u64 a, u64 c) {
    u32 k, K, b, b2;
    const u32 lo = __builtin_addc((u32)a, (u32)c, 0u, &k);
    const u32 hi = __builtin_addc((u32)(a >> 32), (u32)(c >> 32), k, &K);
    u32 r0 = __builtin_subc(lo, 0u, K, &b);
    u32 r1 = __builtin_addc(hi, 0u, K, &b2);
    r1 -= b;
#if defined(__HIP_DEVICE_COMPILE__)
    asm("" : "+v"(r0), "+v"(r1));
#endif
    return ((u64)r1 << 32) | r0;
}

GL_HD u64 fold_al_ah(u64 al, u64 ah) {
#if defined(__HIP_DEVICE_COMPILE__)
    const u64 ah2 = gl::add_u32(ah, (u32)(al >> 32));
#else
    const u64 ah2 = ah + (al >> 32);
#endif
    const u32 x2 = (u32)(ah2 >> 32);
    const u64 base = (ah2 << 32) | (u32)al;
#if defined(__HIP_DEVICE_COMPILE__)
    gl::sg sc, dead;
    u64 r = gl::mad_eps_co(x2, base, sc);
    if (__builtin_expect(sc != 0, 0)) r = gl::mad_eps_co(gl::one_where(sc), r, dead);
    return r;
#else
    const u64 t = base + (u64)x2 * gl::EPS;
    return t < base ? t + gl::EPS : t;
#endif
}

GL_HD void mds_full(u64* s, const unsigned long long* rc, const u32 rows = 0xFFF) {
#if defined(__HIP_DEVICE_COMPILE__)
    u32 l[12], h[12];
    u64 res[12];
#pragma unroll
    for (int i = 0; i < 12; i++) {
        l[i] = (u32)s[i];
        h[i] = (u32)(s[i] >> 32);
    }
#define P2_MDS_T(n, K) "v_mad_u64_u32 %[al], %[d], %[l" #n "], " #K ", %[al]\n\tv_mad_u64_u32 %[ah], %[d], %[h" #n "], " #K ", %[ah]\n\t"
#define P2_MDS_TAIL P2_MDS_T(1, 15) P2_MDS_T(2, 41) P2_MDS_T(3, 16) P2_MDS_T(4, 2) P2_MDS_T(5, 28) P2_MDS_T(6, 13) P2_MDS_T(7, 13) \
                    P2_MDS_T(8, 39) P2_MDS_T(9, 18) P2_MDS_T(10, 34) P2_MDS_T(11, 20)
#define P2_MDS_IN(r)                                                                                                                          \
    [l0] "v"(l[(0 + r) % 12]), [h0] "v"(h[(0 + r) % 12]), [l1] "v"(l[(1 + r) % 12]), [h1] "v"(h[(1 + r) % 12]), [l2] "v"(l[(2 + r) % 12]),     \
        [h2] "v"(h[(2 + r) % 12]), [l3] "v"(l[(3 + r) % 12]), [h3] "v"(h[(3 + r) % 12]), [l4] "v"(l[(4 + r) % 12]), [h4] "v"(h[(4 + r) % 12]), \
        [l5] "v"(l[(5 + r) % 12]), [h5] "v"(h[(5 + r) % 12]), [l6] "v"(l[(6 + r) % 12]), [h6] "v"(h[(6 + r) % 12]), [l7] "v"(l[(7 + r) % 12]), \
        [h7] "v"(h[(7 + r) % 12]), [l8] "v"(l[(8 + r) % 12]), [h8] "v"(h[(8 + r) % 12]), [l9] "v"(l[(9 + r) % 12]), [h9] "v"(h[(9 + r) % 12]), \
        [l10] "v"(l[(10 + r) % 12]), [h10] "v"(h[(10 + r) % 12]), [l11] "v"(l[(11 + r) % 12]), [h11] "v"(h[(11 + r) % 12])
#pragma unroll
    for (int r = 0; r < 12; r++) {
        res[r] = s[r];
        if (!((rows >> r) & 1)) continue;
        u64 al, ah;
        gl::sg dead;
        if (rc) {
            const u64 rl = (u64)(u32)rc[r], rh = (u64)(rc[r] >> 32);
            if (r == 0)
                asm("v_mad_u64_u32 %[al], %[d], %[l0], 17, %[rl]\n\tv_mad_u64_u32 %[ah], %[d], %[h0], 17, %[rh]\n\t" P2_MDS_TAIL
                    "v_mad_u64_u32 %[al], %[d], %[l0], 8, %[al]\n\tv_mad_u64_u32 %[ah], %[d], %[h0], 8, %[ah]"
                    : [al] "=&v"(al), [ah] "=&v"(ah), [d] "=&s"(dead)
                    : [rl] "s"(rl), [rh] "s"(rh), P2_MDS_IN(r));
            else
                asm("v_mad_u64_u32 %[al], %[d], %[l0], 17, %[rl]\n\tv_mad_u64_u32 %[ah], %[d], %[h0], 17, %[rh]\n\t" P2_MDS_TAIL
                    : [al] "=&v"(al), [ah] "=&v"(ah), [d] "=&s"(dead)
                    : [rl] "s"(rl), [rh] "s"(rh), P2_MDS_IN(r));
        } else {
            if (r == 0)
                asm("v_mad_u64_u32 %[al], %[d], %[l0], 17, 0\n\tv_mad_u64_u32 %[ah], %[d], %[h0], 17, 0\n\t" P2_MDS_TAIL
                    "v_mad_u64_u32 %[al], %[d], %[l0], 8, %[al]\n\tv_mad_u64_u32 %[ah], %[d], %[h0], 8, %[ah]"
                    : [al] "=&v"(al), [ah] "=&v"(ah), [d] "=&s"(dead)
                    : P2_MDS_IN(r));
            else
                asm("v_mad_u64_u32 %[al], %[d], %[l0], 17, 0\n\tv_mad_u64_u32 %[ah], %[d], %[h0], 17, 0\n\t" P2_MDS_TAIL
                    : [al] "=&v"(al), [ah] "=&v"(ah), [d] "=&s"(dead)
                    : P2_MDS_IN(r));
        }
        res[r] = fold_al_ah(al, ah);
    }
#pragma unroll
    for (int i = 0; i < 12; i++) s[i] = res[i];
    return;
#endif
    const u32 C[12] = {17, 15, 41, 16, 2, 28, 13, 13, 39, 18, 34, 20};
    u64 lo[12], hi[12], out[12];
#pragma unroll
    for (int i = 0; i < 12; i++) {
        lo[i] = s[i] & gl::EPS;
        hi[i] = s[i] >> 32;
    }
#pragma unroll
    for (int r = 0; r < 12; r++) {
        out[r] = s[r];
        if (!((rows >> r) & 1)) continue;
        u64 al = rc ? (u64)(u32)rc[r] : 0, ah = rc ? (u64)(rc[r] >> 32) : 0;
#pragma unroll
        for (int i = 0; i < 12; i++) {
            int j = (i + r) % 12;
            al += lo[j] * C[i];
            ah += hi[j] * C[i];
        }
        if (r == 0) {
            al += lo[0] * 8;
            ah += hi[0] * 8;
        }
// ... 41 lines not shown

GL_HD void full_round(u64* s, const unsigned long long* rc_next) {
#pragma unroll
    for (int i = 0; i < 12; i++) s[i] = sbox7(s[i]);
    mds_full(s, rc_next);
}

GL_HD u64 mulr_add(u64 a, u64 b, u64 c) {
#if defined(__HIP_DEVICE_COMPILE__)
    return gl::mulr_add_dev<true>(a, b, c);
#else
    unsigned __int128 m = (unsigned __int128)a * b + c;
    return red128((u64)(m >> 64), (u64)m);
#endif
}

GL_HD u64 mulr_add_k(u64 k, u64 b, u64 c) {
#if defined(__HIP_DEVICE_COMPILE__)
    return gl::mulr_add_dev<true, true>(k, b, c);
#else
    return mulr_add(k, b, c);
#endif
}

enum : u32 { FR_GENERAL = 0, FR_ZERO_CAP = 1, FR_ZERO_RATE = 2 };
enum : u32 { ROWS_ALL = 0xFFF, ROWS_DIGEST = 0x00F, ROWS_CAPACITY = 0xF00 };

GL_HD constexpr u32 rows_before_chunk(int m) { return m <= 0 ? 0x00Fu : m >= 8 ? 0xF00u : (0xFFFu & ~((1u << m) - 1u)); }

GL_HD constexpr u32 mds_coef(int r, int j) {
    constexpr u32 C[12] = {17, 15, 41, 16, 2, 28, 13, 13, 39, 18, 34, 20};
    return C[(j - r + 12) % 12] + ((r == 0 && j == 0) ? 8u : 0u);
}

#if defined(__HIP_DEVICE_COMPILE__)
#define P2_FR_T(n) "v_mad_u64_u32 %[al], %[d], %[l" #n "], %[k" #n "], %[al]\n\tv_mad_u64_u32 %[ah], %[d], %[h" #n "], %[k" #n "], %[ah]\n\t"
template <int R>
GL_D void mds_rate_terms(u64& al, u64& ah, const u32* l, const u32* h, u64 rl, u64 rh) {
    gl::sg dead;
    asm("v_mad_u64_u32 %[al], %[d], %[l0], %[k0], %[rl]\n\tv_mad_u64_u32 %[ah], %[d], %[h0], %[k0], %[rh]\n\t"
        P2_FR_T(1) P2_FR_T(2) P2_FR_T(3) P2_FR_T(4) P2_FR_T(5) P2_FR_T(6) "v_mad_u64_u32 %[al], %[d], %[l7], %[k7], %[al]\n\t"
        "v_mad_u64_u32 %[ah], %[d], %[h7], %[k7], %[ah]"
        : [al] "=&v"(al), [ah] "=&v"(ah), [d] "=&s"(dead)
        : [rl] "s"(rl), [rh] "s"(rh), [l0] "v"(l[0]), [h0] "v"(h[0]), [l1] "v"(l[1]), [h1] "v"(h[1]), [l2] "v"(l[2]), [h2] "v"(h[2]),
          [l3] "v"(l[3]), [h3] "v"(h[3]), [l4] "v"(l[4]), [h4] "v"(h[4]), [l5] "v"(l[5]), [h5] "v"(h[5]), [l6] "v"(l[6]), [h6] "v"(h[6]),
          [l7] "v"(l[7]), [h7] "v"(h[7]), [k0] "n"(mds_coef(R, 0)), [k1] "n"(mds_coef(R, 1)), [k2] "n"(mds_coef(R, 2)),
          [k3] "n"(mds_coef(R, 3)), [k4] "n"(mds_coef(R, 4)), [k5] "n"(mds_coef(R, 5)), [k6] "n"(mds_coef(R, 6)), [k7] "n"(mds_coef(R, 7)));
}
template <int R, bool ADDEND>
GL_D void mds_cap_terms(u64& al, u64& ah, const u32* l, const u32* h, u64 rl, u64 rh) {
    gl::sg dead;
#define P2_FR_CAP_IN                                                                                                                      \
    [l8] "v"(l[8]), [h8] "v"(h[8]), [l9] "v"(l[9]), [h9] "v"(h[9]), [l10] "v"(l[10]), [h10] "v"(h[10]), [l11] "v"(l[11]), [h11] "v"(h[11]), \
        [k8] "n"(mds_coef(R, 8)), [k9] "n"(mds_coef(R, 9)), [k10] "n"(mds_coef(R, 10)), [k11] "n"(mds_coef(R, 11))
    if (ADDEND)
        asm("v_mad_u64_u32 %[al], %[d], %[l8], %[k8], %[rl]\n\tv_mad_u64_u32 %[ah], %[d], %[h8], %[k8], %[rh]\n\t"
            P2_FR_T(9) P2_FR_T(10) "v_mad_u64_u32 %[al], %[d], %[l11], %[k11], %[al]\n\t"
            "v_mad_u64_u32 %[ah], %[d], %[h11], %[k11], %[ah]"
            : [al] "=&v"(al), [ah] "=&v"(ah), [d] "=&s"(dead)
            : [rl] "s"(rl), [rh] "s"(rh), P2_FR_CAP_IN);
    else
        asm(P2_FR_T(8) P2_FR_T(9) P2_FR_T(10) "v_mad_u64_u32 %[al], %[d], %[l11], %[k11], %[al]\n\t"
            "v_mad_u64_u32 %[ah], %[d], %[h11], %[k11], %[ah]"
            : [al] "+v"(al), [ah] "+v"(ah), [d] "=&s"(dead)
            : P2_FR_CAP_IN);
#undef P2_FR_CAP_IN
}
#undef P2_FR_T
template <int R>
GL_D u64 first_round_row(const u32 kind, const u32* l, const u32* h, const u64 add) {
    u64 al, ah;
    mds_rate_terms<R>(al, ah, l, h, (u64)(u32)add, add >> 32);
    if (kind != FR_ZERO_CAP) mds_cap_terms<R, false>(al, ah, l, h, 0, 0);
    return fold_al_ah(al, ah);
}
template <int R>
GL_D u64 zero_rate_row(const u32* l, const u32* h, const u64 add) {
    u64 al, ah;
    mds_cap_terms<R, true>(al, ah, l, h, (u64)(u32)add, add >> 32);
    return fold_al_ah(al, ah);
}
#endif

GL_HD void full_round_known(u64* s, const u32 kind, const unsigned long long* pre, const unsigned long long* add) {
#if defined(__HIP_DEVICE_COMPILE__)
    u32 l[12], h[12];
    if (kind == FR_ZERO_RATE) {
#pragma unroll
        for (int i = 8; i < 12; i++) {
            const u64 z = sbox7(pre ? add_wrap(s[i], pre[i]) : s[i]);
            l[i] = (u32)z;
            h[i] = (u32)(z >> 32);
        }
#define P2_FR_ROW(r) s[r] = zero_rate_row<r>(l, h, add[r]);
        P2_FR_ROW(0) P2_FR_ROW(1) P2_FR_ROW(2) P2_FR_ROW(3) P2_FR_ROW(4) P2_FR_ROW(5) P2_FR_ROW(6) P2_FR_ROW(7) P2_FR_ROW(8) P2_FR_ROW(9)
        P2_FR_ROW(10) P2_FR_ROW(11)
#undef P2_FR_ROW
        return;
    }
    if (pre) {
#pragma unroll
        for (int i = 0; i < 8; i++) s[i] = add_wrap(s[i], pre[i]);
    }
#pragma unroll
    for (int i = 0; i < 8; i++) s[i] = sbox7(s[i]);
    if (kind != FR_ZERO_CAP) {
        if (pre) {
#pragma unroll
            for (int i = 8; i < 12; i++) s[i] = add_wrap(s[i], pre[i]);
        }
#pragma unroll
        for (int i = 8; i < 12; i++) s[i] = sbox7(s[i]);
    }
#pragma unroll
    for (int i = 0; i < 12; i++) {
        l[i] = (u32)s[i];
        h[i] = (u32)(s[i] >> 32);
    }
#define P2_FR_ROW(r) s[r] = first_round_row<r>(kind, l, h, add[r]);
    P2_FR_ROW(0) P2_FR_ROW(1) P2_FR_ROW(2) P2_FR_ROW(3) P2_FR_ROW(4) P2_FR_ROW(5) P2_FR_ROW(6) P2_FR_ROW(7) P2_FR_ROW(8) P2_FR_ROW(9)
    P2_FR_ROW(10) P2_FR_ROW(11)
#undef P2_FR_ROW
#else
    const int j0 = kind == FR_ZERO_RATE ? 8 : 0, j1 = kind == FR_ZERO_CAP ? 8 : 12;
    u64 out[12];
    for (int j = j0; j < j1; j++) s[j] = sbox7(pre ? add_wrap(s[j], pre[j]) : s[j]);
    for (int r = 0; r < 12; r++) {
        u64 al = (u32)add[r], ah = add[r] >> 32;
        for (int j = j0; j < j1; j++) {
            al += (s[j] & gl::EPS) * mds_coef(r, j);
            ah += (s[j] >> 32) * mds_coef(r, j);
        }
        out[r] = fold_al_ah(al, ah);
    }
    for (int i = 0; i < 12; i++) s[i] = out[i];
#endif
}
GL_HD const unsigned long long* poseidon_rc() {
#if defined(__HIP_DEVICE_COMPILE__)
    return (const unsigned long long*)gl::D_POSEIDON_RC;
#else
    return (const unsigned long long*)gl::H_POSEIDON_RC;
#endif
}
GL_HD void first_round_any(u64* s, const u32 kind) {
    full_round_known(s, kind, poseidon_rc(), kind == FR_ZERO_CAP ? RC1_ZCAP : kind == FR_ZERO_RATE ? RC1_ZRATE : poseidon_rc() + 12);
}
template <u32 KIND>
GL_HD void first_round(u64* s) {
    static_assert(KIND <= FR_ZERO_RATE, "FR_GENERAL, FR_ZERO_CAP or FR_ZERO_RATE");
    first_round_any(s, KIND);
}

#if defined(__HIP_DEVICE_COMPILE__)
#define P2_PB_T(n) "v_mad_u64_u32 %[al], %[d], %[l" #n "], %[k" #n "], %[al]\n\tv_mad_u64_u32 %[ah], %[d], %[h" #n "], %[k" #n "], %[ah]\n\t"
#define P2_PB_LAST(n) "v_mad_u64_u32 %[al], %[d], %[l" #n "], %[k" #n "], %[al]\n\tv_mad_u64_u32 %[ah], %[d], %[h" #n "], %[k" #n "], %[ah]"
#define P2_PB_IN(n) [l##n] "v"(l[n]), [h##n] "v"(h[n]), [k##n] "s"(c[n])
GL_D u64 block_row0_d2(const u32* l, const u32* h, const u64 t1, const unsigned int* c, const u64 k) {
    const u64 rl = (u64)(u32)k, rh = k >> 32;
    u64 al, ah;
    gl::sg dead;
    asm("v_mad_u64_u32 %[al], %[d], %[lt], 25, %[rl]\n\tv_mad_u64_u32 %[ah], %[d], %[ht], 25, %[rh]\n\t"
        P2_PB_T(0) P2_PB_T(1) P2_PB_T(2) P2_PB_T(3) P2_PB_T(4) P2_PB_LAST(5)
        : [al] "=&v"(al), [ah] "=&v"(ah), [d] "=&s"(dead)
        : [rl] "s"(rl), [rh] "s"(rh), [lt] "v"((u32)t1), [ht] "v"((u32)(t1 >> 32)), P2_PB_IN(0), P2_PB_IN(1), P2_PB_IN(2), P2_PB_IN(3),
          P2_PB_IN(4), P2_PB_IN(5));
    asm(P2_PB_T(6) P2_PB_T(7) P2_PB_T(8) P2_PB_T(9) P2_PB_T(10) P2_PB_LAST(11)
        : [al] "+v"(al), [ah] "+v"(ah), [d] "=&s"(dead)
        : P2_PB_IN(6), P2_PB_IN(7), P2_PB_IN(8), P2_PB_IN(9), P2_PB_IN(10), P2_PB_IN(11));
    return fold_al_ah(al, ah);
}
template <int R>
GL_D u64 block_end_row(const u32* l, const u32* h, const u64 t1, const u64 t2, const unsigned int* e, const u64 k) {
    const u64 rl = (u64)(u32)k, rh = k >> 32;
    const unsigned int* c = e + 1;
    u64 al, ah;
    gl::sg dead;
    asm("v_mad_u64_u32 %[al], %[d], %[lu], %[ku], %[rl]\n\tv_mad_u64_u32 %[ah], %[d], %[hu], %[ku], %[rh]\n\t"
        P2_PB_T(t) P2_PB_T(0) P2_PB_T(1) P2_PB_T(2) P2_PB_T(3) P2_PB_T(4) P2_PB_LAST(5)
        : [al] "=&v"(al), [ah] "=&v"(ah), [d] "=&s"(dead)
        : [rl] "s"(rl), [rh] "s"(rh), [lu] "v"((u32)t2), [hu] "v"((u32)(t2 >> 32)), [ku] "n"(mds_coef(R, 0)), [lt] "v"((u32)t1),
          [ht] "v"((u32)(t1 >> 32)), [kt] "s"(e[0]), P2_PB_IN(0), P2_PB_IN(1), P2_PB_IN(2), P2_PB_IN(3), P2_PB_IN(4), P2_PB_IN(5));
    asm(P2_PB_T(6) P2_PB_T(7) P2_PB_T(8) P2_PB_T(9) P2_PB_T(10) P2_PB_LAST(11)
        : [al] "+v"(al), [ah] "+v"(ah), [d] "=&s"(dead)
        : P2_PB_IN(6), P2_PB_IN(7), P2_PB_IN(8), P2_PB_IN(9), P2_PB_IN(10), P2_PB_IN(11));
    return fold_al_ah(al, ah);
}
#undef P2_PB_T
#undef P2_PB_LAST
#undef P2_PB_IN
#else
GL_HD u64 block_row(const u64* y, const unsigned int* c, const u64 t1, const u32 ct1, const u64 t2, const u32 ct2, const u64 k) {
    u64 al = (u64)(u32)k + (t1 & gl::EPS) * ct1 + (t2 & gl::EPS) * ct2, ah = (k >> 32) + (t1 >> 32) * ct1 + (t2 >> 32) * ct2;
    for (int j = 0; j < 12; j++) {
        al += (y[j] & gl::EPS) * c[j];
        ah += (y[j] >> 32) * c[j];
    }
    return fold_al_ah(al, ah);
}
#endif
GL_HD void block_end(u64* s, const u64 t1, const u64 t2, const unsigned int* e, const unsigned long long* k) {
    u64 res[12];
#if defined(__HIP_DEVICE_COMPILE__)
    u32 l[12], h[12];
#pragma unroll
    for (int i = 0; i < 12; i++) {
        l[i] = (u32)s[i];
        h[i] = (u32)(s[i] >> 32);
    }
#define P2_PB_ROW(r) res[r] = block_end_row<r>(l, h, t1, t2, e + 13 * r, k[r]);
    P2_PB_ROW(0) P2_PB_ROW(1) P2_PB_ROW(2) P2_PB_ROW(3) P2_PB_ROW(4) P2_PB_ROW(5) P2_PB_ROW(6) P2_PB_ROW(7) P2_PB_ROW(8) P2_PB_ROW(9)
    P2_PB_ROW(10) P2_PB_ROW(11)
#undef P2_PB_ROW
#else
    for (int r = 0; r < 12; r++) res[r] = block_row(s, e + 13 * r + 1, t1, e[13 * r], t2, mds_coef(r, 0), k[r]);
#endif
#pragma unroll
    for (int i = 0; i < 12; i++) s[i] = res[i];
}
GL_HD void partial_block(u64* s) {
#pragma nounroll
    for (int b = 0; b < 8; b++) {
        const unsigned long long* K = PB_K + 14 * b;
        const bool three = b < 7;
        s[0] = sbox7(s[0]);
        u64 t1 = 0, t2 = 0;
        if (three) {
            t1 = sbox7(mds_row0(s, K[0]));
#if defined(__HIP_DEVICE_COMPILE__)
            u32 l[12], h[12];
#pragma unroll
            for (int i = 0; i < 12; i++) {
                l[i] = (u32)s[i];
                h[i] = (u32)(s[i] >> 32);
            }
            t2 = sbox7(block_row0_d2(l, h, t1, PB_ROW0_D2, K[1]));
#else
            t2 = sbox7(block_row(s, PB_ROW0_D2, t1, mds_coef(0, 0), 0, 0, K[1]));
#endif
        }
        block_end(s, t1, t2, PB_END + (three ? 0 : 12 * 13), K + 2);
    }
}
GL_HD void middle(u64* s) {
    const unsigned long long* RC = poseidon_rc();
    for (int r = 1; r < 4; r++) full_round(s, RC + 12 * (r + 1));
    partial_block(s);
    for (int r = 26; r < 29; r++) full_round(s, RC + 12 * (r + 1));
}

GL_HD void last_round_any(u64* s, const u32 rows) {
#pragma unroll
    for (int i = 0; i < 12; i++) s[i] = sbox7(s[i]);
    mds_full(s, PF_ZERO12, rows);
#pragma unroll
    for (int i = 0; i < 12; i++)
        if ((rows >> i) & 1) s[i] = canon(s[i]);
}
template <u32 ROWS>
GL_HD void last_round(u64* s) {
    static_assert(ROWS != 0 && ROWS <= ROWS_ALL, "a mask of output words 0..11");
    last_round_any(s, ROWS);
}

GL_HD void permute_known_any(u64* s, const u32 kind, const u32 rows) {
    const unsigned long long* RC = poseidon_rc();
    const unsigned long long* add0 = kind == FR_ZERO_CAP ? RC1_ZCAP : kind == FR_ZERO_RATE ? RC1_ZRATE : RC + 12;
#pragma nounroll
    for (int r = 0; r < 4; r++) full_round_known(s, r == 0 ? kind : (u32)FR_GENERAL, r == 0 ? RC : nullptr, r == 0 ? add0 : RC + 12 * (r + 1));
    partial_block(s);
#pragma nounroll
    for (int r = 26; r < 30; r++) {
#pragma unroll
        for (int i = 0; i < 12; i++) s[i] = sbox7(s[i]);
        mds_full(s, r < 29 ? RC + 12 * (r + 1) : PF_ZERO12, r < 29 ? (u32)ROWS_ALL : rows);
    }
#pragma unroll
    for (int i = 0; i < 12; i++)
        if ((rows >> i) & 1) s[i] = canon(s[i]);
}
template <u32 KIND, u32 ROWS>
GL_HD void permute_known(u64* s) {
    static_assert(KIND <= FR_ZERO_RATE && ROWS != 0 && ROWS <= ROWS_ALL, "FR_* and a mask of output words 0..11");
    permute_known_any(s, KIND, ROWS);
}

GL_HD void poseidon(u64* s) {
    const unsigned long long* RC = poseidon_rc();
#pragma unroll
    for (int i = 0; i < 12; i++) s[i] = add_wrap(s[i], RC[i]);
    for (int r = 0; r < 4; r++) full_round(s, RC + 12 * (r + 1));
    partial_block(s);
    for (int r = 26; r < 29; r++) full_round(s, RC + 12 * (r + 1));
    full_round(s, nullptr);
#pragma unroll
    for (int i = 0; i < 12; i++) s[i] = canon(s[i]);
}

GL_HD u64 mds_row0_terms(const u64* s, u64 rc) {
#if defined(__HIP_DEVICE_COMPILE__)
    {
        u64 al = gl::madk_s<17>((u32)s[0], (u64)(u32)rc), ah = gl::madk_s<17>((u32)(s[0] >> 32), rc >> 32);
#define P2_MDS_TERM(i, K)                       \
    al = gl::madk<K>((u32)s[i], al);            \
    ah = gl::madk<K>((u32)(s[i] >> 32), ah);
        P2_MDS_TERM(1, 15) P2_MDS_TERM(2, 41) P2_MDS_TERM(3, 16) P2_MDS_TERM(4, 2) P2_MDS_TERM(5, 28) P2_MDS_TERM(6, 13)
        P2_MDS_TERM(7, 13) P2_MDS_TERM(8, 39) P2_MDS_TERM(9, 18) P2_MDS_TERM(10, 34) P2_MDS_TERM(11, 20) P2_MDS_TERM(0, 8)
#undef P2_MDS_TERM
        return fold_al_ah(al, ah);
    }
#endif
    return mds_row0(s, rc);
}
GL_HD void partial_block_sparse(u64* s) {
    {
        u64 z[12];
#pragma unroll
        for (int i = 0; i < 12; i++) z[i] = sbox7(s[i]);
#pragma nounroll
        for (int r = 0; r < 11; r++) {
            Acc a;
            a.init();
#pragma unroll
            for (int c = 0; c < 12; c++) a.fma_k(PF_E[r * 12 + c], z[c]);
            s[1 + r] = a.reduce();
        }
        s[0] = mds_row0_terms(z, PF_A[0]);
    }
    for (int i = 0; i < 22; i++) {
        u64 s0 = sbox7(s[0]);
        Acc a;
        a.init();
        a.e01 = i < 21 ? PF_A[i + 1] : PF_RC26[0];
        a.fma_small(25, s0);
#pragma unroll
        for (int j = 0; j < 11; j++) a.fma_k(PF_WHAT[i * 11 + j], s[1 + j]);
#pragma unroll
        for (int j = 0; j < 11; j++) s[1 + j] = mulr_add_k(PF_V[i * 11 + j], s0, s[1 + j]);
        s[0] = a.reduce();
    }
#pragma unroll
    for (int j = 1; j < 12; j++) s[j] = add_wrap(s[j], PF_RC26[j]);
}
GL_HD void poseidon_sparse(u64* s) {
    const unsigned long long* RC = poseidon_rc();
#pragma unroll
    for (int i = 0; i < 12; i++) s[i] = add_wrap(s[i], RC[i]);
    for (int r = 0; r < 3; r++) full_round(s, RC + 12 * (r + 1));
    partial_block_sparse(s);
    for (int r = 26; r < 29; r++) full_round(s, RC + 12 * (r + 1));
    full_round(s, nullptr);
#pragma unroll
    for (int i = 0; i < 12; i++) s[i] = canon(s[i]);
}

GL_HD u32 sponge_first_kind(int c0, int width, int live) {
    return c0 == 0 ? (u32)FR_ZERO_CAP : (c0 >= live && c0 + 8 <= width) ? (u32)FR_ZERO_RATE : (u32)FR_GENERAL;
}
GL_HD void sponge_permute(u64* s, int c0, int width, int live) {
    permute_known_any(s, sponge_first_kind(c0, width, live), rows_before_chunk(width - (c0 + 8)));
}
GL_HD void two_to_one_permute(u64* s) {
    permute_known<FR_ZERO_CAP, ROWS_DIGEST>(s);
}

#if defined(__HIPCC__)
__device__ __forceinline__ u64 shfl64(u64 v, int src_lane) { return (u64)__shfl((unsigned long long)v, src_lane, 64); }
__device__ inline u64 poseidon_coop(u64 w, const u32 i ) {
    const int lane = (int)(threadIdx.x & 63), gbase = lane & ~15;
    const bool live = i < 12;
    const u32 ii = live ? i : 0;
    const unsigned long long* RC = (const unsigned long long*)gl::D_POSEIDON_RC;
    auto mds = [&](u64 z, u64 rc) -> u64 {
        const u32 C[12] = {17, 15, 41, 16, 2, 28, 13, 13, 39, 18, 34, 20};
        u64 al = (u32)rc, ah = rc >> 32;
#pragma unroll
        for (int k = 0; k < 12; k++) {
            u32 src = i + k;
            src = src >= 12 ? src - 12 : src;
            const u64 x = shfl64(z, gbase + (int)(src & 15));
            const u32 c = C[k] + ((k == 0 && i == 0) ? 8u : 0u);
            al += (x & gl::EPS) * c;
            ah += (x >> 32) * c;
        }
        return fold_al_ah(al, ah);
    };
    w = live ? add_wrap(w, RC[ii]) : 0;
    for (int r = 0; r < 3; r++) w = mds(sbox7(w), live ? RC[12 * (r + 1) + ii] : 0);
    {
        const u64 z = sbox7(w);
        const u64 row0 = mds(z, i == 0 ? PF_A[0] : 0);
        const u32 er = (live && i >= 1) ? i - 1 : 0;
        Acc a;
        a.init();
#pragma unroll
        for (int c = 0; c < 12; c++) a.fma(PF_E[er * 12 + c], shfl64(z, gbase + c));
        const u64 rowe = a.reduce();
        w = i == 0 ? row0 : (live ? rowe : 0);
    }
    for (int pr = 0; pr < 22; pr++) {
        const u64 z0 = shfl64(sbox7(w), gbase);
        const u32 cj = (live && i >= 1) ? pr * 11 + (i - 1) : 0;
        const u64 coef = i == 0 ? 25 : (live ? PF_WHAT[cj] : 0);
        u64 term = canon(mulr(coef, i == 0 ? z0 : w));
#pragma unroll
        for (int d = 1; d < 16; d <<= 1) term = gl::add(term, shfl64(term, lane ^ d));
        const u64 s0n = gl::add(term, pr < 21 ? PF_A[pr + 1] : PF_RC26[0]);
        const u64 wj = mulr_add((live && i >= 1) ? PF_V[cj] : 0, z0, w);
        w = i == 0 ? s0n : wj;
    }
    if (live && i >= 1) w = add_wrap(w, PF_RC26[ii]);
    for (int r = 26; r < 29; r++) w = mds(sbox7(w), live ? RC[12 * (r + 1) + ii] : 0);
    w = mds(sbox7(w), 0);
    return live ? canon(w) : 0;
}
#endif

}
```

plonky2-aes_amd/csrc/poseidon_fast.inc:

```
P2F_DECL const unsigned long long PF_A[22] = {
    0x3cc3f892184df408ULL, 0x6754826bf0555feaULL, 0x07f136d86fe52ec6ULL, 0xcc31104c136e624cULL,
    0xe75f601068e70acaULL, 0x27bb558ab181ed5eULL, 0xe0593bc645a018abULL, 0xa7ef236c2c5f0e1fULL,
    0x2f2ed40f0e211d79ULL, 0x65b0ab09bec15af9ULL, 0x28f0f3bb03d3d776ULL, 0xb60fb82205a86176ULL,
    0x6685ae6e5db8023dULL, 0x9b2390b07020a27cULL, 0xc3607e7232b11cefULL, 0xf618ae7058499e24ULL,
    0xc18226dd334780c2ULL, 0xb57bff1387506176ULL, 0xec2475152d5a08ffULL, 0x04df43ffd0b458ffULL,
    0x10f46236adcc3e98ULL, 0x52588ae3575e2ce9ULL,
};
P2F_DECL const unsigned long long PF_WHAT[22 * 11] = {
    0x3d999c961b7c63b0ULL, 0x814e82efcd172529ULL, 0x2421e5d236704588ULL, 0x887af7d4dd482328ULL,
    0xa5e9c291f6119b27ULL, 0xbdc52b2676a4b4aaULL, 0x64832009d29bcf57ULL, 0x09c4155174a552ccULL,
    0x463f9ee03d290810ULL, 0xc810936e64982542ULL, 0x043b1c289f7bc3acULL, 0x673655aae8be5a8bULL,
    0xd510fe714f39fa10ULL, 0x2c68a099b51c9e73ULL, 0xa667bfa9aa96999dULL, 0x4d67e72f063e2108ULL,
    0xf84dde3e6acda179ULL, 0x40f9cc8c08f80981ULL, 0x5ead032050097142ULL, 0x6591b02092d671bbULL,
    0x00e18c71963dd1b7ULL, 0x8a21bcd24a14218aULL, 0x202800f4addbdc87ULL, 0xe4b5bdb1cc3504ffULL,
    0xbe32b32a825596e7ULL, 0x8e0f68c5dc223b9aULL, 0x58022d9e1c256ce3ULL, 0x584d29227aa073acULL,
    0x8b9352ad04bef9e7ULL, 0xaead42a3f445ecbfULL, 0x3c667a1d833a3ccaULL, 0xda6f61838efa1ffeULL,
    0xe8f749470bd7c446ULL, 0xc5b85bab9e5b3869ULL, 0x45245258aec51cf7ULL, 0x16e6b8e68b931830ULL,
    0xe2ae0f051418112cULL, 0x0470e26a0093a65bULL, 0x6bef71973a8146edULL, 0x119265be51812dafULL,
    0xb0be7356254bea2eULL, 0x8584defff7589bd7ULL, 0x3c5fe4aeb1fb52baULL, 0x9e7cd88acf543a5eULL,
    0x179be4bba87f0a8cULL, 0xacf63d95d8887355ULL, 0x6696670196b0074fULL, 0xd99ddf1fe75085f9ULL,
    0xc2597881fef0283bULL, 0xcf48395ee6c54f14ULL, 0x15226a8e4cd8d3b6ULL, 0xc053297389af5d3bULL,
    0x2c08893f0d1580e2ULL, 0x0ed3cbcff6fcc5baULL, 0xc82f510ecf81f6d0ULL, 0x94b06183acb715ccULL,
    0x500392ed0d431137ULL, 0x861cc95ad5c86323ULL, 0x05830a443f86c4acULL, 0x3b68225874a20a7cULL,
    0x10b3309838e236fbULL, 0x9b77fc8bcd559e2cULL, 0xbdecf5e0cb9cb213ULL, 0x30276f1221ace5faULL,
// ... 135 lines not shown
    0x81c44e9699915693ULL, 0x63c9679d8572a867ULL, 0x462269e4b04620a5ULL, 0xd499fcbf63fbd266ULL,
    0xe04ea1957ad8305cULL, 0x383dd77e07998487ULL, 0xdb6945a20d277091ULL, 0x60c33ebd1e023f0aULL,
    0x72af70cdcb99214fULL, 0x9b6e5164ed35d878ULL, 0x97f9b7d2cfc2ade5ULL, 0xe95c10ae32e05085ULL,
    0x2c4916605e3dea58ULL, 0xa6fdb8ebccc51667ULL, 0x3743057c07a5dbfaULL, 0xe6fdf23648931b99ULL,
    0xde2a0516f8c9d943ULL, 0xfa9db0de2d852e7aULL, 0x2dc10fce3233f443ULL, 0xd267254bea1097f4ULL,
    0xe3ef40eacc6ff78dULL, 0x6fadc9347faeee81ULL, 0x9b6e5164ed35d878ULL, 0x17f9202c16676b2fULL,
    0xeb4c0ce280c3e935ULL, 0x66c8bab2096cfd38ULL, 0x59ccc4d5184bc93aULL, 0x605a82c52b5ad2f1ULL,
    0x727eca45c8d7bb71ULL, 0x7a5cf5b7b922e946ULL, 0x819f2c14a8366b1fULL, 0x817bd8a7869ed1b5ULL,
};
P2F_DECL const unsigned long long PF_RC26[12] = {
    0x5405cc09b3ff0c06ULL, 0xe14dc071ace29846ULL, 0xbb56729c7877aa9eULL, 0x474fb5726a0068f3ULL,
    0x2629b158383529bfULL, 0xe1cabee6fa7a9532ULL, 0xced9e7d28e6a6de9ULL, 0xd0fd98f1e129850fULL,
    0x9689ab45a6d09dd7ULL, 0xba9673a4862f9848ULL, 0xa5c3a8c0fcbdbd41ULL, 0x8f4411a1226beb35ULL,
};
P2F_DECL const unsigned long long RC1_ZCAP[12] = {
    0x62cfea8e55341db8ULL, 0x53ae0d422f8cc6efULL, 0xac29b888aeef84d6ULL, 0x90cc491f71b5fd4eULL,
    0x638cd97d1f14244cULL, 0xf3fc76291302124dULL, 0xc57293658eb53e57ULL, 0x60bea017e5f8e6a2ULL,
    0x54c44c3971082de9ULL, 0xb7d39352c39511f2ULL, 0xb39c19ddc44cc469ULL, 0x301a0d485cf527f6ULL,
};
P2F_DECL const unsigned long long RC1_ZRATE[12] = {
    0x69bb5cd44bcf58fdULL, 0xae595cd0ad28486cULL, 0xf49966579bfa11d0ULL, 0x2e32abc0199d1d4aULL,
    0xc09b96778f4c42bbULL, 0x50f528d8574ab731ULL, 0x6b7c3093a8fc635fULL, 0xd5d9cf526048a682ULL,
    0xae3bfab5edd3203bULL, 0xb10f872338efe4c1ULL, 0xa200f67ad423ef8fULL, 0x143e446176468f75ULL,
};
P2F_DECL const unsigned int PB_ROW0_D2[12] = {
    5017u, 5577u, 3889u, 4968u, 6188u, 4656u, 4977u, 5755u, 4895u, 4430u, 5968u, 4864u,
};
P2F_DECL const unsigned int PB_END[2 * 12 * 13] = {
    5017u, 1259209u, 1214817u, 1089681u, 1265600u, 1256596u, 1145944u, 1308833u, 1199363u, 1101695u, 1264278u, 1095368u, 1177368u,
    4864u, 1177368u, 1245100u, 1098072u, 1190716u, 1300784u, 1133572u, 1206472u, 1279668u, 1065320u, 1209572u, 1138800u, 1175868u,
    5968u, 1095368u, 1078368u, 1034088u, 1115568u, 1149856u, 1093360u, 1118088u, 1092896u, 1040696u, 1097728u, 966368u, 1138800u,
    4430u, 1264278u, 1205802u, 1101998u, 1269500u, 1268360u, 1156924u, 1283798u, 1207246u, 1100850u, 1297432u, 1097728u, 1209572u,
    4895u, 1101695u, 1134223u, 997679u, 1083496u, 1182252u, 1052008u, 1106983u, 1138253u, 964737u, 1100850u, 1040696u, 1065320u,
    5755u, 1199363u, 1229703u, 1139523u, 1217028u, 1273780u, 1206844u, 1246827u, 1220837u, 1138253u, 1207246u, 1092896u, 1279668u,
    4977u, 1308833u, 1215705u, 1128169u, 1287344u, 1286388u, 1160104u, 1302425u, 1246827u, 1106983u, 1283798u, 1118088u, 1206472u,
    4656u, 1145944u, 1229284u, 1046872u, 1170628u, 1251568u, 1103164u, 1160104u, 1206844u, 1052008u, 1156924u, 1093360u, 1133572u,
    6188u, 1256596u, 1269180u, 1199540u, 1256688u, 1367024u, 1251568u, 1286388u, 1273780u, 1182252u, 1268360u, 1149856u, 1300784u,
    4968u, 1265600u, 1204572u, 1096600u, 1299092u, 1256688u, 1170628u, 1287344u, 1217028u, 1083496u, 1269500u, 1115568u, 1190716u,
    3889u, 1089681u, 1137505u, 1024929u, 1096600u, 1199540u, 1046872u, 1128169u, 1139523u, 997679u, 1101998u, 1034088u, 1098072u,
    5577u, 1214817u, 1202205u, 1137505u, 1204572u, 1269180u, 1229284u, 1215705u, 1229703u, 1134223u, 1205802u, 1078368u, 1245100u,
    0u, 25u, 15u, 41u, 16u, 2u, 28u, 13u, 13u, 39u, 18u, 34u, 20u,
    0u, 20u, 17u, 15u, 41u, 16u, 2u, 28u, 13u, 13u, 39u, 18u, 34u,
    0u, 34u, 20u, 17u, 15u, 41u, 16u, 2u, 28u, 13u, 13u, 39u, 18u,
    0u, 18u, 34u, 20u, 17u, 15u, 41u, 16u, 2u, 28u, 13u, 13u, 39u,
    0u, 39u, 18u, 34u, 20u, 17u, 15u, 41u, 16u, 2u, 28u, 13u, 13u,
    0u, 13u, 39u, 18u, 34u, 20u, 17u, 15u, 41u, 16u, 2u, 28u, 13u,
    0u, 13u, 13u, 39u, 18u, 34u, 20u, 17u, 15u, 41u, 16u, 2u, 28u,
    0u, 28u, 13u, 13u, 39u, 18u, 34u, 20u, 17u, 15u, 41u, 16u, 2u,
    0u, 2u, 28u, 13u, 13u, 39u, 18u, 34u, 20u, 17u, 15u, 41u, 16u,
    0u, 16u, 2u, 28u, 13u, 13u, 39u, 18u, 34u, 20u, 17u, 15u, 41u,
    0u, 41u, 16u, 2u, 28u, 13u, 13u, 39u, 18u, 34u, 20u, 17u, 15u,
    0u, 15u, 41u, 16u, 2u, 28u, 13u, 13u, 39u, 18u, 34u, 20u, 17u,
};
P2F_DECL const unsigned long long PB_K[8 * 14] = {
    0x7131aa45268d7d8cULL, 0xf1417c86de0778d0ULL, 0xbe56ca781ef1f717ULL, 0x9a8644b3a029077bULL,
    0x52b02192268817e7ULL, 0x0abc5297582f33a3ULL, 0xe54f22ee7990679aULL, 0xa469d6aea2518f18ULL,
    0xbb1b667d37b273ccULL, 0x3c358ffba2a4519dULL, 0xbe01b370410f63faULL, 0xd5ba62f78b5714f8ULL,
    0x20bf71b9d89243c8ULL, 0x7af4c52b70c921f3ULL, 0x7159cd30c3ac118eULL, 0x3efc75806ff4f0e2ULL,
    0x854e26e7fd0a553bULL, 0x6e2d494da714d050ULL, 0x15536d53b9653dfdULL, 0xdc1b35793f2ac720ULL,
    0x371b585ed71b5368ULL, 0x4ca149f23e2320abULL, 0x7c4fd5da0194e8f8ULL, 0x44d6d6eaa5ac26e0ULL,
    0x6e4712cfe6151b8fULL, 0x44680366e0558d8aULL, 0x0839ba7c6da2cab4ULL, 0x586a9fb8e2327e99ULL,
    0x30a4680593258387ULL, 0xc750352d9b604341ULL, 0xd6b93cc966e3abc2ULL, 0x36ee51b452289282ULL,
    0x1bb20c3a458f7d4dULL, 0x1ffdfb49ac80cdfaULL, 0x0fa800e4298022d5ULL, 0xdbf976a1b996bbc1ULL,
    0x225b39a176f2d4d5ULL, 0xa45d5e6b69082198ULL, 0x3809a401fa675720ULL, 0xc2e6704cb5c50370ULL,
    0x1d5e6b2865fbbcd7ULL, 0x463334214bb5e49fULL, 0x775005982d74d7f7ULL, 0x3fe3eee08a73b798ULL,
    0x66809a1bd77d2177ULL, 0x25bd84ce6b7b1a7bULL, 0xde59fdea3047b692ULL, 0x75fb00dd10178af1ULL,
    0x46556f5c2d9c33ceULL, 0x699471c4bd25de10ULL, 0x2a6ebf09632059cbULL, 0xa17b58038b8c3be9ULL,
    0x8fc747be82537744ULL, 0x790d302d429da700ULL, 0x2c41991afdf0055eULL, 0x32f3edefc6bfc0abULL,
    0xdd611f1000c17442ULL, 0xe44c4dd5fac93576ULL, 0x15f154a2d41b033fULL, 0xd1795c6e29688609ULL,
    0xf3267319116c6ec1ULL, 0x74ee383cad93b9ccULL, 0xca17dcb4fcd44819ULL, 0x28eb017c36869a7eULL,
    0xd8c39810c49a303dULL, 0x91a5e951f4f8d367ULL, 0xb14f64de8c856749ULL, 0x0e0f4582c32305f1ULL,
    0x5def8c2e86f7685aULL, 0x166054a2c28f9600ULL, 0xe89cd854d5d01d33ULL, 0x44e8d81a988250a0ULL,
    0x6fa1906153a3e603ULL, 0x2f29361714b1b0f2ULL, 0xfcb0885586303ee1ULL, 0x2e17c5d7e4dde9b3ULL,
    0x58d3390853fe1c65ULL, 0xaebfdda047d8dcedULL, 0x675d6c7ae5747ec6ULL, 0x27732879d25def23ULL,
    0xb8d35c9d5ccc86e5ULL, 0x4fe2afbe081bafe9ULL, 0xfd1e3e36d78e7686ULL, 0xb18169e4f66def9cULL,
    0xde122bebe9a39368ULL, 0xa7529fb85d2e95d9ULL, 0xab5eb4de7870a682ULL, 0x6ae79d56fa73f523ULL,
    0xf650f4f4357ef8a2ULL, 0xa140ca8818f720d6ULL, 0xbc531094fe62eb20ULL, 0xb2b726df19911c1dULL,
    0x77c73890c761c075ULL, 0x5d605fb1cc7702dbULL, 0x2965bb9926a636beULL, 0x530cc0067855c471ULL,
    0xabc50207c93c9b30ULL, 0x063f5cc2eb195297ULL, 0x0000000000000000ULL, 0x0000000000000000ULL,
    0x475cd3205a3bdcdeULL, 0x18a42105c31b7e88ULL, 0x023e7414af663068ULL, 0x15147108121967d7ULL,
    0xe4a3dff1d7d6fef9ULL, 0x01a8d1a588085737ULL, 0x11b4c74eda62beefULL, 0xe587cc0d69a73346ULL,
    0x1ff7327017aa2a6eULL, 0x594e29c42473d06bULL, 0xf6f31db1899b12d5ULL, 0xc02ac5e47312d3caULL,
};
```

plonky2-aes_amd/csrc/prover_gpu.hip:

```cpp
#include <hip/hip_runtime.h>
#include <chrono>
#include <cstring>

#include <algorithm>
#include <map>
#include <mutex>
#include <random>
#include <string>
#include <thread>

#include "capi_common.h"
#include "os_random.h"
#include "kernels.h"
#include "kernels2.h"
#include "kernels_compress.h"
#include "kernels_keccak.h"
#include "kernels_witness_io.h"
#include "verifier.h"

using namespace p2;
using namespace p2k;

#define HIPCHECK(expr)                                                                          \
    do {                                                                                        \
// ... 2185 lines not shown
            const u64 e = (t & 2) ? (mm << 32) : (gl::P - mm), f = (t & 2) ? (1ull << 32) : (1ull << 48);
            if (gl::mul(e, f) != gl::mul_ref(e, f)) b++;
        }
    }
    u64 s0[12], s1[12];
    for (int k = 0; k < 12; k++) {
        s1[k] = (t & 3) == 3 ? rnd() : rnd() % gl::P;
        s0[k] = s1[k] % gl::P;
    }
    gl::poseidon(s0);
    glf::poseidon(s1);
    for (int k = 0; k < 12; k++) b += s0[k] != s1[k];
    if (b) atomicAdd(bad, b);
}
__global__ __launch_bounds__(64) void k_selftest_coop(unsigned long long* bad, u64 seed) {
    const u32 t = blockIdx.x * blockDim.x + threadIdx.x, grp = t >> 4, i = t & 15;
    u64 st[12];
    u64 x = (seed | 1) + 0x9E3779B97F4A7C15ull * (grp + 1);
    for (int k = 0; k < 12; k++) {
        x ^= x << 13;
        x ^= x >> 7;
        x ^= x << 17;
        st[k] = (grp & 7) == 0 ? (k & 1 ? gl::P - 1 : 0) : x % gl::P;
    }
    u64 mine = 0;
    for (int k = 0; k < 12; k++)
        if ((u32)k == i) mine = st[k];
    const u64 got = glf::poseidon_coop(mine, i);
    gl::poseidon(st);
    u64 want = 0;
    for (int k = 0; k < 12; k++)
        if ((u32)k == i) want = st[k];
    if (got != want) atomicAdd(bad, 1ull);
}
}

int p2_selftest_device(uint64_t seed, size_t threads, int device) {
    if (hipSetDevice(device) != hipSuccess) return set_error("no such HIP device"), -P2_ERR_HIP;
    Allocs mem;
    unsigned long long* d = nullptr;
    if (dalloc(mem, &d, 1) || hipMemset(d, 0, 8) != hipSuccess) return set_error("hipMalloc failed"), -P2_ERR_HIP;
    hipLaunchKernelGGL(p2k::k_selftest, dim3((u32)((threads + 255) / 256)), dim3(256), 0, 0, d, (u64)seed, threads);
    hipLaunchKernelGGL(p2k::k_selftest_coop, dim3((u32)std::min<size_t>(std::max<size_t>(threads / 64, 1), 4096)), dim3(64), 0, 0, d, (u64)seed);
    unsigned long long h = 0;
    if (hipError_t e = hipMemcpy(&h, d, 8, hipMemcpyDeviceToHost)) return set_error(hipGetErrorString(e)), -P2_ERR_HIP;
    return (int)std::min<unsigned long long>(h, 0x7FFFFFFF);
}

int p2_gpu_poseidon(uint64_t* states, size_t n_perm, int device) {
    if (int rc = pick_device(device)) return rc;
    Allocs mem;
    u64* d;
    if (upload(mem, &d, (const u64*)states, n_perm * 12)) return P2_ERR_HIP;
    hipLaunchKernelGGL(k_poseidon_states, g1(n_perm, 256), dim3(256), 0, 0, d, n_perm);
    HIPCHECK(hipGetLastError());
    HIPCHECK(hipMemcpy(states, d, n_perm * 96, hipMemcpyDeviceToHost));
    return P2_OK;
}
int p2_gpu_hash_leaves(const uint64_t* data, size_t cols, size_t active_cols, size_t num_leaves, size_t batch, uint64_t* digests, int device) {
    if (cols == 0 || cols > (1u << 20) || num_leaves == 0 || batch == 0 || batch > 65535) return set_error("shape out of range"), P2_ERR_INVALID;
    if (int rc = pick_device(device)) return rc;
    const size_t stored = std::min(active_cols, cols), in_words = std::max<size_t>(stored, 1) * num_leaves;
    Allocs mem;
    u64 *d_in, *d_out;
    if (dalloc(mem, &d_in, batch * in_words) || dalloc(mem, &d_out, batch * num_leaves * 4)) return P2_ERR_HIP;
    HIPCHECK(hipMemcpy(d_in, data, batch * stored * num_leaves * 8, hipMemcpyHostToDevice));
    hipLaunchKernelGGL(k_hash_leaves, g1(num_leaves, 256, (u32)batch), dim3(256), 0, 0, d_in, (int)cols, (int)active_cols, num_leaves, stored * num_leaves, num_leaves,
                       d_out, num_leaves * 4);
    HIPCHECK(hipGetLastError());
    HIPCHECK(hipMemcpy(digests, d_out, batch * num_leaves * 32, hipMemcpyDeviceToHost));
    return P2_OK;
}
int p2_gpu_partial_rounds(uint64_t* states, size_t count, int device) {
    if (count == 0 || count > (1u << 24)) return set_error("count out of range"), P2_ERR_INVALID;
    if (int rc = pick_device(device)) return rc;
    Allocs mem;
    u64* d;
    if (upload(mem, &d, (const u64*)states, count * 12)) return P2_ERR_HIP;
    hipLaunchKernelGGL(k_partial_rounds, g1(count, 256), dim3(256), 0, 0, d, count);
    HIPCHECK(hipGetLastError());
    HIPCHECK(hipMemcpy(states, d, count * 96, hipMemcpyDeviceToHost));
    return P2_OK;
}
int p2_gpu_merkle_level(const uint64_t* child, size_t num_parents, size_t batch, uint64_t* parent, int device) {
    if (num_parents == 0 || batch == 0 || batch > 65535) return set_error("shape out of range"), P2_ERR_INVALID;
    if (int rc = pick_device(device)) return rc;
    const size_t stride = 8 * num_parents;
    Allocs mem;
    u64 *d_in, *d_out;
    if (upload(mem, &d_in, (const u64*)child, batch * stride) || dalloc(mem, &d_out, batch * stride)) return P2_ERR_HIP;
    hipLaunchKernelGGL(k_merkle_level, g1(num_parents, 256, (u32)batch), dim3(256), 0, 0, d_in, d_out, num_parents, stride);
    HIPCHECK(hipGetLastError());
    for (size_t b = 0; b < batch; b++) HIPCHECK(hipMemcpy(parent + b * 4 * num_parents, d_out + b * stride, num_parents * 32, hipMemcpyDeviceToHost));
    return P2_OK;
}
int p2_gpu_hash_fri_leaves(const uint64_t* vals, size_t len, int arity, size_t batch, uint64_t* digests, int device) {
    if (arity < 1 || arity > 64 || len == 0 || len % (size_t)arity || batch == 0 || batch > 65535) return set_error("shape out of range"), P2_ERR_INVALID;
    if (int rc = pick_device(device)) return rc;
    const size_t leaves = len / (size_t)arity;
    Allocs mem;
    u64 *d_in, *d_out;
    if (upload(mem, &d_in, (const u64*)vals, batch * 2 * len) || dalloc(mem, &d_out, batch * leaves * 4)) return P2_ERR_HIP;
    hipLaunchKernelGGL(k_hash_fri_leaves, g1(leaves, 256, (u32)batch), dim3(256), 0, 0, d_in, len, 2 * len, arity, d_out, leaves * 4);
    HIPCHECK(hipGetLastError());
    HIPCHECK(hipMemcpy(digests, d_out, batch * leaves * 32, hipMemcpyDeviceToHost));
    return P2_OK;
}
struct PrimCtx {
    Lane lane;
    Domain dom;
    Allocs mem;
    int init(int device, int degree_bits) {
        if (int rc = pick_device(device)) return rc;
        dom.logn = (u32)degree_bits;
        HIPCHECK(hipStreamCreate(&lane.stream));
        HIPCHECK(raise_ntt_lds_limits());
        const size_t n = dom.n();
        std::vector<u64> twf(n), twi(n);
        u64 w = gl::root_of_unity(degree_bits), wi = gl::inv(w), x = 1, xi = 1;
        for (size_t i = 0; i < n; i++) {
            twf[i] = x;
            twi[i] = xi;
            x = gl::mul(x, w);
            xi = gl::mul(xi, wi);
        }
        if (upload(mem, &dom.d_tw_fwd_full, twf.data(), n) || upload(mem, &dom.d_tw_inv_full, twi.data(), n)) return P2_ERR_HIP;
        dom.d_tw_fwd = dom.d_tw_fwd_full;
        dom.d_tw_inv = dom.d_tw_inv_full;
        if (ensure_pass1_table(lane, dom, mem, dom.d_tw_fwd_full, dom.logn) || ensure_pass1_table(lane, dom, mem, dom.d_tw_inv_full, dom.logn)) return P2_ERR_HIP;
        std::vector<u64> bases(8);
        u64 wl = gl::root_of_unity(degree_bits + 3);
        for (u32 j = 0; j < 8; j++) bases[j] = gl::mul(gl::MULT_GEN, gl::pow(wl, j));
        u64* d_b;
        if (upload(mem, &d_b, bases.data(), 8)) return P2_ERR_HIP;
        if (dalloc(mem, &dom.d_shift_pows[0], 8 * n)) return P2_ERR_HIP;
        hipLaunchKernelGGL(k_pow_table, g1(n, 256, 8), dim3(256), 0, lane.stream, dom.d_shift_pows[0], d_b, (u32)n, (u64)1);
        HIPCHECK(hipGetLastError());
        return 0;
    }
    ~PrimCtx() {
        if (lane.stream) (void)hipStreamSynchronize(lane.stream);
        if (lane.stream) (void)hipStreamDestroy(lane.stream);
    }
};
int p2_gpu_intt(const uint64_t* values, size_t cols, int degree_bits, uint64_t* coeffs, int device) {
    if (degree_bits < 1 || degree_bits > 22) return set_error("degree_bits must be in 1..22"), P2_ERR_INVALID;
    PrimCtx ctx;
    if (int rc = ctx.init(device, degree_bits)) return rc;
    const size_t n = ctx.dom.n();
    u64 *d_in, *d_out, *d_scratch;
    if (upload(ctx.mem, &d_in, (const u64*)values, cols * n) || dalloc(ctx.mem, &d_out, cols * n) || dalloc(ctx.mem, &d_scratch, cols * n)) return P2_ERR_HIP;
    if (intt_cols(ctx.lane, ctx.dom, d_in, d_out, (u32)cols, 0, 1, d_scratch, 0)) return P2_ERR_HIP;
    HIPCHECK(hipStreamSynchronize(ctx.lane.stream));
    HIPCHECK(hipMemcpy(coeffs, d_out, cols * n * 8, hipMemcpyDeviceToHost));
    return P2_OK;
}
int p2_gpu_lde(const uint64_t* coeffs, size_t cols, int degree_bits, int rate_bits, uint64_t* lde, int device) {
    if (degree_bits < 1 || degree_bits > 22 || rate_bits != 3) return set_error("degree_bits must be in 1..22 and rate_bits 3"), P2_ERR_INVALID;
    PrimCtx ctx;
    if (int rc = ctx.init(device, degree_bits)) return rc;
    const size_t n = ctx.dom.n();
    u64 *d_in, *d_out;
    if (upload(ctx.mem, &d_in, (const u64*)coeffs, cols * n) || dalloc(ctx.mem, &d_out, cols * 8 * n)) return P2_ERR_HIP;
    if (lde_cols(ctx.lane, ctx.dom, d_in, 0, d_out, 0, (u32)cols, 0, 1)) return P2_ERR_HIP;
    HIPCHECK(hipStreamSynchronize(ctx.lane.stream));
    HIPCHECK(hipMemcpy(lde, d_out, cols * 8 * n * 8, hipMemcpyDeviceToHost));
// ... 54 lines not shown
```

Before: 713.2.

## Merge last full-round MDS into partial-round blocks of Poseidon

Result: faster. 753.2 (median of 6 runs) (+5.6%).

```diff
diff --git a/bindings/plonky2-hip/src/ffi.rs b/bindings/plonky2-hip/src/ffi.rs
--- a/bindings/plonky2-hip/src/ffi.rs
+++ b/bindings/plonky2-hip/src/ffi.rs
@@ -106,6 +106,7 @@
     pub fn p2_selftest_device(seed: u64, threads: usize, device: c_int) -> c_int;
     pub fn p2_host_poseidon_known(states: *mut u64, n_perm: usize, kind: c_int, rows: u32, parts: c_int) -> c_int;
     pub fn p2_host_partial_rounds(states: *mut u64, count: usize) -> c_int;
+    pub fn p2_host_merged_middle(states: *mut u64, count: usize) -> c_int;
     pub fn p2_host_hash_leaves(data: *const u64, cols: usize, active_cols: usize, num_leaves: usize, digests: *mut u64) -> c_int;
     pub fn p2_native_gf_2_8_mul(a: u8, b: u8) -> u8;
     pub fn p2_native_aes_key_expansion(key: *const u8, nk: c_int, nr: c_int, out: *mut u8);
@@ -162,6 +163,7 @@
     pub fn p2_gpu_merkle_cap_hasher(cols_major: *const u64, cols: usize, num_leaves: usize, cap_height: c_int, hasher: c_int, cap: *mut u64, device: c_int) -> c_int;
     pub fn p2_gpu_hash_leaves(data: *const u64, cols: usize, active_cols: usize, num_leaves: usize, batch: usize, digests: *mut u64, device: c_int) -> c_int;
     pub fn p2_gpu_partial_rounds(states: *mut u64, count: usize, device: c_int) -> c_int;
+    pub fn p2_gpu_merged_middle(states: *mut u64, count: usize, device: c_int) -> c_int;
     pub fn p2_gpu_merkle_level(child: *const u64, num_parents: usize, batch: usize, parent: *mut u64, device: c_int) -> c_int;
     pub fn p2_gpu_hash_fri_leaves(vals: *const u64, len: usize, arity: c_int, batch: usize, digests: *mut u64, device: c_int) -> c_int;
     pub fn p2_circuit_debug_read(a0: *mut P2Circuit, name: *const c_char, index: usize, out: *mut u64, cap: usize, n_written: *mut usize) -> c_int;
diff --git a/include/p2aes.h b/include/p2aes.h
--- a/include/p2aes.h
+++ b/include/p2aes.h
@@ -132,6 +132,7 @@
 int p2_selftest_device(uint64_t seed, size_t threads, int device);
 int p2_host_poseidon_known(uint64_t* states, size_t n_perm, int kind, uint32_t rows, int parts);
 int p2_host_partial_rounds(uint64_t* states, size_t count);
+int p2_host_merged_middle(uint64_t* states, size_t count);
 int p2_host_hash_leaves(const uint64_t* data, size_t cols, size_t active_cols, size_t num_leaves, uint64_t* digests);
 
 uint8_t p2_native_gf_2_8_mul(uint8_t a, uint8_t b);
@@ -251,6 +252,7 @@
 int p2_gpu_merkle_cap_hasher(const uint64_t* cols_major, size_t cols, size_t num_leaves, int cap_height, int hasher, uint64_t* cap, int device);
 int p2_gpu_hash_leaves(const uint64_t* data, size_t cols, size_t active_cols, size_t num_leaves, size_t batch, uint64_t* digests, int device);
 int p2_gpu_partial_rounds(uint64_t* states, size_t count, int device);
+int p2_gpu_merged_middle(uint64_t* states, size_t count, int device);
 int p2_gpu_merkle_level(const uint64_t* child, size_t num_parents, size_t batch, uint64_t* parent, int device);
 int p2_gpu_hash_fri_leaves(const uint64_t* vals, size_t len, int arity, size_t batch, uint64_t* digests, int device);
 int p2_circuit_debug_read(p2_circuit*, const char* name, size_t index, uint64_t* out, size_t cap, size_t* n_written);
diff --git a/plonky2-aes_amd/api.py b/plonky2-aes_amd/api.py
--- a/plonky2-aes_amd/api.py
+++ b/plonky2-aes_amd/api.py
@@ -243,6 +243,8 @@
         "p2_gpu_poseidon": (C.c_int, [u64p, sz, C.c_int]),
         "p2_host_partial_rounds": (C.c_int, [u64p, sz]),
         "p2_gpu_partial_rounds": (C.c_int, [u64p, sz, C.c_int]),
+        "p2_host_merged_middle": (C.c_int, [u64p, sz]),
+        "p2_gpu_merged_middle": (C.c_int, [u64p, sz, C.c_int]),
         "p2_gpu_lde": (C.c_int, [u64p, sz, C.c_int, C.c_int, u64p, C.c_int]),
         "p2_gpu_intt": (C.c_int, [u64p, sz, C.c_int, u64p, C.c_int]),
         "p2_gpu_merkle_cap": (C.c_int, [u64p, sz, sz, C.c_int, u64p, C.c_int]),
diff --git a/plonky2-aes_amd/csrc/capi_host.cpp b/plonky2-aes_amd/csrc/capi_host.cpp
--- a/plonky2-aes_amd/csrc/capi_host.cpp
+++ b/plonky2-aes_amd/csrc/capi_host.cpp
@@ -515,6 +515,10 @@
 }
 int p2_host_partial_rounds(uint64_t* states, size_t count) {
     for (size_t i = 0; i < count; i++) glf::partial_block(states + 12 * i);
+    return P2_OK;
+}
+int p2_host_merged_middle(uint64_t* states, size_t count) {
+    for (size_t i = 0; i < count; i++) glf::merged_middle(states + 12 * i);
     return P2_OK;
 }
 int p2_host_hash_leaves(const uint64_t* data, size_t cols, size_t active_cols, size_t num_leaves, uint64_t* digests) {
diff --git a/plonky2-aes_amd/csrc/kernels.h b/plonky2-aes_amd/csrc/kernels.h
--- a/plonky2-aes_amd/csrc/kernels.h
+++ b/plonky2-aes_amd/csrc/kernels.h
@@ -145,6 +145,15 @@
     u64 st[12];
     for (int k = 0; k < 12; k++) st[k] = states[12 * i + k];
     glf::partial_block(st);
+    for (int k = 0; k < 12; k++) states[12 * i + k] = st[k];
+}
+
+__global__ __launch_bounds__(256) P2_HASH_WAVES void k_merged_middle(u64* states, size_t n) {
+    size_t i = (size_t)blockIdx.x * blockDim.x + threadIdx.x;
+    if (i >= n) return;
+    u64 st[12];
+    for (int k = 0; k < 12; k++) st[k] = states[12 * i + k];
+    glf::merged_middle(st);
     for (int k = 0; k < 12; k++) states[12 * i + k] = st[k];
 }
 
@@ -1165,7 +1174,7 @@
         u64 r[12];
 #pragma unroll
         for (int i = 0; i < 12; i++) r[i] = ((u32)i == pos) ? cand : sh[i];
-        glf::poseidon(r);
+        glf::poseidon<false>(r);
         if ((r[7] >> (64 - pow_bits)) == 0) atomicMin(&best[p], (unsigned long long)cand);
     }
 }
diff --git a/plonky2-aes_amd/csrc/poseidon_fast.h b/plonky2-aes_amd/csrc/poseidon_fast.h
--- a/plonky2-aes_amd/csrc/poseidon_fast.h
+++ b/plonky2-aes_amd/csrc/poseidon_fast.h
@@ -167,6 +167,7 @@
     return ((u64)r1 << 32) | r0;
 }
 
+template <bool ALWAYS = false>
 GL_HD u64 fold_al_ah(u64 al, u64 ah) {
 #if defined(__HIP_DEVICE_COMPILE__)
     const u64 ah2 = gl::add_u32(ah, (u32)(al >> 32));
@@ -177,6 +178,16 @@
     const u64 base = (ah2 << 32) | (u32)al;
 #if defined(__HIP_DEVICE_COMPILE__)
     gl::sg sc, dead;
+    if (ALWAYS) {
+        u64 r = base;
+        u32 c01 = x2;
+        asm("v_mad_u64_u32 %[r], %[sc], %[c], -1, %[r]\n\t"
+            "s_nop 1\n\t"
+            "v_cndmask_b32_e64 %[c], 0, 1, %[sc]\n\t"
+            "v_mad_u64_u32 %[r], %[d], %[c], -1, %[r]"
+            : [r] "+v"(r), [c] "+v"(c01), [sc] "=&s"(sc), [d] "=&s"(dead));
+        return r;
+    }
     u64 r = gl::mad_eps_co(x2, base, sc);
     if (__builtin_expect(sc != 0, 0)) r = gl::mad_eps_co(gl::one_where(sc), r, dead);
     return r;
@@ -384,41 +395,47 @@
 }
 #endif
 
-GL_HD void full_round_known(u64* s, const u32 kind, const unsigned long long* pre, const unsigned long long* add) {
+GL_HD void sbox_layer_known(u64* s, const u32 kind, const unsigned long long* pre) {
+#if defined(__HIP_DEVICE_COMPILE__)
+    if (kind == FR_ZERO_RATE) {
+#pragma unroll
+        for (int i = 8; i < 12; i++) s[i] = sbox7(pre ? add_wrap(s[i], pre[i]) : s[i]);
+        return;
+    }
+    if (pre) {
+#pragma unroll
+        for (int i = 0; i < 8; i++) s[i] = add_wrap(s[i], pre[i]);
+    }
+#pragma unroll
+    for (int i = 0; i < 8; i++) s[i] = sbox7(s[i]);
+    if (kind != FR_ZERO_CAP) {
+        if (pre) {
+#pragma unroll
+            for (int i = 8; i < 12; i++) s[i] = add_wrap(s[i], pre[i]);
+        }
+#pragma unroll
+        for (int i = 8; i < 12; i++) s[i] = sbox7(s[i]);
+    }
+#else
+    const int j0 = kind == FR_ZERO_RATE ? 8 : 0, j1 = kind == FR_ZERO_CAP ? 8 : 12;
+    for (int j = j0; j < j1; j++) s[j] = sbox7(pre ? add_wrap(s[j], pre[j]) : s[j]);
+#endif
+}
+GL_HD void linear_layer_known(u64* s, const u32 kind, const unsigned long long* add) {
 #if defined(__HIP_DEVICE_COMPILE__)
     u32 l[12], h[12];
+#pragma unroll
+    for (int i = 0; i < 12; i++) {
+        l[i] = (u32)s[i];
+        h[i] = (u32)(s[i] >> 32);
+    }
     if (kind == FR_ZERO_RATE) {
-#pragma unroll
-        for (int i = 8; i < 12; i++) {
-            const u64 z = sbox7(pre ? add_wrap(s[i], pre[i]) : s[i]);
-            l[i] = (u32)z;
-            h[i] = (u32)(z >> 32);
-        }
 #define P2_FR_ROW(r) s[r] = zero_rate_row<r>(l, h, add[r]);
         P2_FR_ROW(0) P2_FR_ROW(1) P2_FR_ROW(2) P2_FR_ROW(3) P2_FR_ROW(4) P2_FR_ROW(5) P2_FR_ROW(6) P2_FR_ROW(7) P2_FR_ROW(8) P2_FR_ROW(9)
         P2_FR_ROW(10) P2_FR_ROW(11)
 #undef P2_FR_ROW
         return;
     }
-    if (pre) {
-#pragma unroll
-        for (int i = 0; i < 8; i++) s[i] = add_wrap(s[i], pre[i]);
-    }
-#pragma unroll
-    for (int i = 0; i < 8; i++) s[i] = sbox7(s[i]);
-    if (kind != FR_ZERO_CAP) {
-        if (pre) {
-#pragma unroll
-            for (int i = 8; i < 12; i++) s[i] = add_wrap(s[i], pre[i]);
-        }
-#pragma unroll
-        for (int i = 8; i < 12; i++) s[i] = sbox7(s[i]);
-    }
-#pragma unroll
-    for (int i = 0; i < 12; i++) {
-        l[i] = (u32)s[i];
-        h[i] = (u32)(s[i] >> 32);
-    }
 #define P2_FR_ROW(r) s[r] = first_round_row<r>(kind, l, h, add[r]);
     P2_FR_ROW(0) P2_FR_ROW(1) P2_FR_ROW(2) P2_FR_ROW(3) P2_FR_ROW(4) P2_FR_ROW(5) P2_FR_ROW(6) P2_FR_ROW(7) P2_FR_ROW(8) P2_FR_ROW(9)
     P2_FR_ROW(10) P2_FR_ROW(11)
@@ -426,7 +443,6 @@
 #else
     const int j0 = kind == FR_ZERO_RATE ? 8 : 0, j1 = kind == FR_ZERO_CAP ? 8 : 12;
     u64 out[12];
-    for (int j = j0; j < j1; j++) s[j] = sbox7(pre ? add_wrap(s[j], pre[j]) : s[j]);
     for (int r = 0; r < 12; r++) {
         u64 al = (u32)add[r], ah = add[r] >> 32;
         for (int j = j0; j < j1; j++) {
@@ -437,6 +453,10 @@
     }
     for (int i = 0; i < 12; i++) s[i] = out[i];
 #endif
+}
+GL_HD void full_round_known(u64* s, const u32 kind, const unsigned long long* pre, const unsigned long long* add) {
+    sbox_layer_known(s, kind, pre);
+    linear_layer_known(s, kind, add);
 }
 GL_HD const unsigned long long* poseidon_rc() {
 #if defined(__HIP_DEVICE_COMPILE__)
@@ -488,6 +508,39 @@
         : P2_PB_IN(6), P2_PB_IN(7), P2_PB_IN(8), P2_PB_IN(9), P2_PB_IN(10), P2_PB_IN(11));
     return fold_al_ah(al, ah);
 }
+static_assert((PM_ALWAYS_ROW0 & 3) == 0, "mds_row0 and block_row0_d2 fold with the rare-carry branch");
+GL_D u64 merged_row0_d3(const u32* l, const u32* h, const u64 t1, const u64 t2, const unsigned int* e, const u64 k) {
+    const u64 rl = (u64)(u32)k, rh = k >> 32;
+    const unsigned int* c = e + 1;
+    u64 al, ah;
+    gl::sg dead;
+    asm("v_mad_u64_u32 %[al], %[d], %[lu], 25, %[rl]\n\tv_mad_u64_u32 %[ah], %[d], %[hu], 25, %[rh]\n\t"
+        P2_PB_T(t) P2_PB_T(0) P2_PB_T(1) P2_PB_T(2) P2_PB_T(3) P2_PB_T(4) P2_PB_LAST(5)
+        : [al] "=&v"(al), [ah] "=&v"(ah), [d] "=&s"(dead)
+        : [rl] "s"(rl), [rh] "s"(rh), [lu] "v"((u32)t2), [hu] "v"((u32)(t2 >> 32)), [lt] "v"((u32)t1), [ht] "v"((u32)(t1 >> 32)),
+          [kt] "s"(e[0]), P2_PB_IN(0), P2_PB_IN(1), P2_PB_IN(2), P2_PB_IN(3), P2_PB_IN(4), P2_PB_IN(5));
+    asm(P2_PB_T(6) P2_PB_T(7) P2_PB_T(8) P2_PB_T(9) P2_PB_T(10) P2_PB_LAST(11)
+        : [al] "+v"(al), [ah] "+v"(ah), [d] "=&s"(dead)
+        : P2_PB_IN(6), P2_PB_IN(7), P2_PB_IN(8), P2_PB_IN(9), P2_PB_IN(10), P2_PB_IN(11));
+    return fold_al_ah<((PM_ALWAYS_ROW0 >> 2) & 1) != 0>(al, ah);
+}
+template <int R>
+GL_D u64 merged_end_row(const u32* l, const u32* h, const u64 t1, const u64 t2, const u64 t3, const unsigned int* e, const u64 k) {
+    const u64 rl = (u64)(u32)k, rh = k >> 32;
+    const unsigned int* c = e + 2;
+    u64 al, ah;
+    gl::sg dead;
+    asm("v_mad_u64_u32 %[al], %[d], %[lu], %[ku], %[rl]\n\tv_mad_u64_u32 %[ah], %[d], %[hu], %[ku], %[rh]\n\t"
+        P2_PB_T(t) P2_PB_T(v) P2_PB_T(0) P2_PB_T(1) P2_PB_T(2) P2_PB_T(3) P2_PB_LAST(4)
+        : [al] "=&v"(al), [ah] "=&v"(ah), [d] "=&s"(dead)
+        : [rl] "s"(rl), [rh] "s"(rh), [lu] "v"((u32)t3), [hu] "v"((u32)(t3 >> 32)), [ku] "n"(mds_coef(R, 0)), [lt] "v"((u32)t1),
+          [ht] "v"((u32)(t1 >> 32)), [kt] "s"(e[0]), [lv] "v"((u32)t2), [hv] "v"((u32)(t2 >> 32)), [kv] "s"(e[1]), P2_PB_IN(0), P2_PB_IN(1),
+          P2_PB_IN(2), P2_PB_IN(3), P2_PB_IN(4));
+    asm(P2_PB_T(5) P2_PB_T(6) P2_PB_T(7) P2_PB_T(8) P2_PB_T(9) P2_PB_T(10) P2_PB_LAST(11)
+        : [al] "+v"(al), [ah] "+v"(ah), [d] "=&s"(dead)
+        : P2_PB_IN(5), P2_PB_IN(6), P2_PB_IN(7), P2_PB_IN(8), P2_PB_IN(9), P2_PB_IN(10), P2_PB_IN(11));
+    return fold_al_ah<(((PM_ALWAYS_END4 | PM_ALWAYS_END3) >> R) & 1) != 0>(al, ah);
+}
 #undef P2_PB_T
 #undef P2_PB_LAST
 #undef P2_PB_IN
@@ -499,6 +552,16 @@
         ah += (y[j] >> 32) * c[j];
     }
     return fold_al_ah(al, ah);
+}
+GL_HD u64 merged_row(const u64* y, const unsigned int* c, const u64 t1, const u32 ct1, const u64 t2, const u32 ct2, const u64 t3, const u32 ct3,
+                     const u64 k) {
+    u64 al = (u64)(u32)k + (t1 & gl::EPS) * ct1 + (t2 & gl::EPS) * ct2 + (t3 & gl::EPS) * ct3;
+    u64 ah = (k >> 32) + (t1 >> 32) * ct1 + (t2 >> 32) * ct2 + (t3 >> 32) * ct3;
+    for (int j = 0; j < 12; j++) {
+        al += (y[j] & gl::EPS) * c[j];
+        ah += (y[j] >> 32) * c[j];
+    }
+    return fold_al_ah<true>(al, ah);
 }
 #endif
 GL_HD void block_end(u64* s, const u64 t1, const u64 t2, const unsigned int* e, const unsigned long long* k) {
@@ -544,10 +607,56 @@
         block_end(s, t1, t2, PB_END + (three ? 0 : 12 * 13), K + 2);
     }
 }
+
+GL_HD void merged_end(u64* s, const u64 t1, const u64 t2, const u64 t3, const unsigned int* e, const unsigned long long* k) {
+    u64 res[12];
+#if defined(__HIP_DEVICE_COMPILE__)
+    u32 l[12], h[12];
+#pragma unroll
+    for (int i = 0; i < 12; i++) {
+        l[i] = (u32)s[i];
+        h[i] = (u32)(s[i] >> 32);
+    }
+#define P2_PM_ROW(r) res[r] = merged_end_row<r>(l, h, t1, t2, t3, e + 14 * r, k[r]);
+    P2_PM_ROW(0) P2_PM_ROW(1) P2_PM_ROW(2) P2_PM_ROW(3) P2_PM_ROW(4) P2_PM_ROW(5) P2_PM_ROW(6) P2_PM_ROW(7) P2_PM_ROW(8) P2_PM_ROW(9)
+    P2_PM_ROW(10) P2_PM_ROW(11)
+#undef P2_PM_ROW
+#else
+    for (int r = 0; r < 12; r++) res[r] = merged_row(s, e + 14 * r + 2, t1, e[14 * r], t2, e[14 * r + 1], t3, mds_coef(r, 0), k[r]);
+#endif
+#pragma unroll
+    for (int i = 0; i < 12; i++) s[i] = res[i];
+}
+GL_HD void merged_middle(u64* s) {
+#pragma nounroll
+    for (int b = 0; b < 6; b++) {
+        const unsigned long long* K = PM_K + 15 * b;
+        const bool four = PM_DEPTH[b] == 4;
+        if (b) s[0] = sbox7(s[0]);
+        const u64 t1 = sbox7(mds_row0(s, K[0]));
+        u64 t3 = 0;
+#if defined(__HIP_DEVICE_COMPILE__)
+        u32 l[12], h[12];
+#pragma unroll
+        for (int i = 0; i < 12; i++) {
+            l[i] = (u32)s[i];
+            h[i] = (u32)(s[i] >> 32);
+        }
+        const u64 t2 = sbox7(block_row0_d2(l, h, t1, PB_ROW0_D2, K[1]));
+        if (four) t3 = sbox7(merged_row0_d3(l, h, t1, t2, PM_ROW0_D3, K[2]));
+#else
+        const u64 t2 = sbox7(block_row(s, PB_ROW0_D2, t1, mds_coef(0, 0), 0, 0, K[1]));
+        if (four) t3 = sbox7(merged_row(s, PM_ROW0_D3 + 1, t1, PM_ROW0_D3[0], t2, mds_coef(0, 0), 0, 0, K[2]));
+#endif
+        merged_end(s, t1, t2, t3, PM_END + (four ? 0 : 12 * 14), K + 3);
+    }
+}
 GL_HD void middle(u64* s) {
     const unsigned long long* RC = poseidon_rc();
-    for (int r = 1; r < 4; r++) full_round(s, RC + 12 * (r + 1));
-    partial_block(s);
+    for (int r = 1; r < 3; r++) full_round(s, RC + 12 * (r + 1));
+#pragma unroll
+    for (int i = 0; i < 12; i++) s[i] = sbox7(s[i]);
+    merged_middle(s);
     for (int r = 26; r < 29; r++) full_round(s, RC + 12 * (r + 1));
 }
 
@@ -565,12 +674,23 @@
     last_round_any(s, ROWS);
 }
 
+template <bool OWN_SBOX3 = false>
 GL_HD void permute_known_any(u64* s, const u32 kind, const u32 rows) {
     const unsigned long long* RC = poseidon_rc();
     const unsigned long long* add0 = kind == FR_ZERO_CAP ? RC1_ZCAP : kind == FR_ZERO_RATE ? RC1_ZRATE : RC + 12;
+    if (OWN_SBOX3) {
 #pragma nounroll
-    for (int r = 0; r < 4; r++) full_round_known(s, r == 0 ? kind : (u32)FR_GENERAL, r == 0 ? RC : nullptr, r == 0 ? add0 : RC + 12 * (r + 1));
-    partial_block(s);
+        for (int r = 0; r < 3; r++) full_round_known(s, r == 0 ? kind : (u32)FR_GENERAL, r == 0 ? RC : nullptr, r == 0 ? add0 : RC + 12 * (r + 1));
+#pragma unroll
+        for (int i = 0; i < 12; i++) s[i] = sbox7(s[i]);
+    } else {
+#pragma nounroll
+        for (int r = 0; r < 4; r++) {
+            if (r) linear_layer_known(s, r == 1 ? kind : (u32)FR_GENERAL, r == 1 ? add0 : RC + 12 * r);
+            sbox_layer_known(s, r == 0 ? kind : (u32)FR_GENERAL, r == 0 ? RC : nullptr);
+        }
+    }
+    merged_middle(s);
 #pragma nounroll
     for (int r = 26; r < 30; r++) {
 #pragma unroll
@@ -587,12 +707,22 @@
     permute_known_any(s, KIND, ROWS);
 }
 
+template <bool MERGED = true>
 GL_HD void poseidon(u64* s) {
     const unsigned long long* RC = poseidon_rc();
 #pragma unroll
     for (int i = 0; i < 12; i++) s[i] = add_wrap(s[i], RC[i]);
-    for (int r = 0; r < 4; r++) full_round(s, RC + 12 * (r + 1));
-    partial_block(s);
+    if (MERGED) {
+        for (int r = 0; r < 4; r++) {
+#pragma unroll
+            for (int i = 0; i < 12; i++) s[i] = sbox7(s[i]);
+            if (r < 3) mds_full(s, RC + 12 * (r + 1));
+        }
+        merged_middle(s);
+    } else {
+        for (int r = 0; r < 4; r++) full_round(s, RC + 12 * (r + 1));
+        partial_block(s);
+    }
     for (int r = 26; r < 29; r++) full_round(s, RC + 12 * (r + 1));
     full_round(s, nullptr);
 #pragma unroll
@@ -660,7 +790,7 @@
     return c0 == 0 ? (u32)FR_ZERO_CAP : (c0 >= live && c0 + 8 <= width) ? (u32)FR_ZERO_RATE : (u32)FR_GENERAL;
 }
 GL_HD void sponge_permute(u64* s, int c0, int width, int live) {
-    permute_known_any(s, sponge_first_kind(c0, width, live), rows_before_chunk(width - (c0 + 8)));
+    permute_known_any<true>(s, sponge_first_kind(c0, width, live), rows_before_chunk(width - (c0 + 8)));
 }
 GL_HD void two_to_one_permute(u64* s) {
     permute_known<FR_ZERO_CAP, ROWS_DIGEST>(s);
diff --git a/plonky2-aes_amd/csrc/poseidon_fast.inc b/plonky2-aes_amd/csrc/poseidon_fast.inc
--- a/plonky2-aes_amd/csrc/poseidon_fast.inc
+++ b/plonky2-aes_amd/csrc/poseidon_fast.inc
@@ -241,3 +241,63 @@
     0xe4a3dff1d7d6fef9ULL, 0x01a8d1a588085737ULL, 0x11b4c74eda62beefULL, 0xe587cc0d69a73346ULL,
     0x1ff7327017aa2a6eULL, 0x594e29c42473d06bULL, 0xf6f31db1899b12d5ULL, 0xc02ac5e47312d3caULL,
 };
+P2F_DECL const unsigned int PM_DEPTH[6] = {
+    4u, 4u, 4u, 4u, 4u, 3u,
+};
+P2F_DECL const unsigned int PM_ROW0_D3[13] = {
+    5017u, 1259209u, 1214817u, 1089681u, 1265600u, 1256596u, 1145944u, 1308833u, 1199363u, 1101695u, 1264278u, 1095368u, 1177368u,
+};
+P2F_DECL const unsigned int PM_END[2 * 12 * 14] = {
+    1259209u, 5017u, 283630249u, 284566993u, 262796737u, 285878768u, 300075668u, 275722040u, 289630625u, 286599123u, 260345679u, 285544326u, 257349000u, 286463800u,
+    1177368u, 4864u, 286463800u, 282235216u, 258285752u, 287754760u, 296642752u, 271739096u, 290242168u, 285243280u, 255387080u, 288070216u, 256952416u, 280233128u,
+    1095368u, 5968u, 257349000u, 262512200u, 237074008u, 258744368u, 274793680u, 248706720u, 262157000u, 263724888u, 233727656u, 259401088u, 237865872u, 256952416u,
+    1264278u, 4430u, 285544326u, 286610446u, 264109942u, 286776120u, 301535656u, 277918552u, 290923062u, 289640266u, 261097450u, 287370636u, 259401088u, 288070216u,
+    1101695u, 4895u, 260345679u, 257114743u, 235238039u, 261741392u, 269863068u, 246789448u, 263978423u, 259853957u, 232686297u, 261097450u, 233727656u, 255387080u,
+    1199363u, 5755u, 286599123u, 291387251u, 262947499u, 288415880u, 304933852u, 275072448u, 291813275u, 293035161u, 259853957u, 289640266u, 263724888u, 285243280u,
+    1308833u, 4977u, 289630625u, 289457257u, 266660569u, 290692048u, 304990452u, 280934520u, 294150169u, 291813275u, 263978423u, 290923062u, 262157000u, 290242168u,
+    1145944u, 4656u, 275722040u, 273698848u, 249385784u, 278089464u, 286678400u, 261972648u, 280934520u, 275072448u, 246789448u, 277918552u, 248706720u, 271739096u,
+    1256596u, 6188u, 300075668u, 302363636u, 274294564u, 300774864u, 317240928u, 286678400u, 304990452u, 304933852u, 269863068u, 301535656u, 274793680u, 296642752u,
+    1265600u, 4968u, 285878768u, 286955896u, 263433136u, 287698696u, 300774864u, 278089464u, 290692048u, 288415880u, 261741392u, 286776120u, 258744368u, 287754760u,
+    1089681u, 3889u, 262796737u, 260725657u, 238321913u, 263433136u, 274294564u, 249385784u, 266660569u, 262947499u, 235238039u, 264109942u, 237074008u, 258285752u,
+    1214817u, 5577u, 284566993u, 289193489u, 260725657u, 286955896u, 302363636u, 273698848u, 289457257u, 291387251u, 257114743u, 286610446u, 262512200u, 282235216u,
+    5017u, 25u, 1259209u, 1214817u, 1089681u, 1265600u, 1256596u, 1145944u, 1308833u, 1199363u, 1101695u, 1264278u, 1095368u, 1177368u,
+    4864u, 20u, 1177368u, 1245100u, 1098072u, 1190716u, 1300784u, 1133572u, 1206472u, 1279668u, 1065320u, 1209572u, 1138800u, 1175868u,
+    5968u, 34u, 1095368u, 1078368u, 1034088u, 1115568u, 1149856u, 1093360u, 1118088u, 1092896u, 1040696u, 1097728u, 966368u, 1138800u,
+    4430u, 18u, 1264278u, 1205802u, 1101998u, 1269500u, 1268360u, 1156924u, 1283798u, 1207246u, 1100850u, 1297432u, 1097728u, 1209572u,
+    4895u, 39u, 1101695u, 1134223u, 997679u, 1083496u, 1182252u, 1052008u, 1106983u, 1138253u, 964737u, 1100850u, 1040696u, 1065320u,
+    5755u, 13u, 1199363u, 1229703u, 1139523u, 1217028u, 1273780u, 1206844u, 1246827u, 1220837u, 1138253u, 1207246u, 1092896u, 1279668u,
+    4977u, 13u, 1308833u, 1215705u, 1128169u, 1287344u, 1286388u, 1160104u, 1302425u, 1246827u, 1106983u, 1283798u, 1118088u, 1206472u,
+    4656u, 28u, 1145944u, 1229284u, 1046872u, 1170628u, 1251568u, 1103164u, 1160104u, 1206844u, 1052008u, 1156924u, 1093360u, 1133572u,
+    6188u, 2u, 1256596u, 1269180u, 1199540u, 1256688u, 1367024u, 1251568u, 1286388u, 1273780u, 1182252u, 1268360u, 1149856u, 1300784u,
+    4968u, 16u, 1265600u, 1204572u, 1096600u, 1299092u, 1256688u, 1170628u, 1287344u, 1217028u, 1083496u, 1269500u, 1115568u, 1190716u,
+    3889u, 41u, 1089681u, 1137505u, 1024929u, 1096600u, 1199540u, 1046872u, 1128169u, 1139523u, 997679u, 1101998u, 1034088u, 1098072u,
+    5577u, 15u, 1214817u, 1202205u, 1137505u, 1204572u, 1269180u, 1229284u, 1215705u, 1229703u, 1134223u, 1205802u, 1078368u, 1245100u,
+};
+P2F_DECL const unsigned long long PM_K[6 * 15] = {
+    0x3cc3f892184df408ULL, 0x6754826bf0555feaULL, 0x07f136d86fe52ec6ULL, 0xcc31104c136e624cULL,
+    0x43b63edb69a1eaacULL, 0x561bc802d7a4d433ULL, 0x85ede3dfa9edfb95ULL, 0xdc38d480924d4386ULL,
+    0xc0e1b2a6a2ab6614ULL, 0x0c3475f550e70a40ULL, 0x768f4c939c84f564ULL, 0xcf3541e232efa58fULL,
+    0x7b3f72490b711d9dULL, 0x887e00e77b43b8d8ULL, 0x0695112e44c24ca7ULL, 0x7159cd30c3ac118eULL,
+    0x3efc75806ff4f0e2ULL, 0x854e26e7fd0a553bULL, 0x0c5074f008691549ULL, 0x7f07cb01952ceb60ULL,
+    0x6a5c79acfed4e507ULL, 0x9d0e5100cbd3f8c1ULL, 0x250a0abe1905e39bULL, 0x0be4a3e95fd07360ULL,
+    0x48def01a8c813278ULL, 0x6969ce54b27ce6b0ULL, 0x51a31975f368450aULL, 0xa704363d4d548e68ULL,
+    0xfdf3a27d8b419e19ULL, 0xe159b1c5b2a1203fULL, 0x15a16a8a8322d458ULL, 0x6539261ddcbcac24ULL,
+    0x79a874245ae7c29cULL, 0xbd7ff03dea9a4885ULL, 0x0eb9953b5e9e26aaULL, 0xc9cfebaa705f6f8bULL,
+    0x96b0c5aaae262753ULL, 0x1237ac16517f532fULL, 0xe9bca9cad77cc1aeULL, 0xba9eb92af3180cf1ULL,
+    0xfc5e6b8fc930a92fULL, 0xcf27496bdb8fbc41ULL, 0x8cb8aa18207198a7ULL, 0x568656b73859787bULL,
+    0x75e0ae608496f268ULL, 0x0c49366bb25e8513ULL, 0x726c2a38b33372eaULL, 0xbca82b9035dfed26ULL,
+    0xc68df5b2962d9be9ULL, 0x0f176f067b99ee1aULL, 0xc0f0936e34655243ULL, 0x2508faae65bb028bULL,
+    0xb8df24970b3de2c0ULL, 0x1aeeea0d94b72efdULL, 0x6cf13b1c5c02d2feULL, 0x6dcd8d74982d5b50ULL,
+    0x2f45c7125ec029b1ULL, 0x5ae39ab597e617fbULL, 0xf0e6e3ee02c125d7ULL, 0xbab12ee36b95632eULL,
+    0xe89cd854d5d01d33ULL, 0x44e8d81a988250a0ULL, 0x6fa1906153a3e603ULL, 0x4cbccb995ba6f700ULL,
+    0xc63c85fbdf7a5283ULL, 0xb5d4e65307748b0dULL, 0x60b47ac209791987ULL, 0x1c490008b1d8910cULL,
+    0xbd78becf9c5c007cULL, 0xa9d1dc81d35069a6ULL, 0x3e58e0e6d689a75dULL, 0x5f42929eed11d322ULL,
+    0x3635444ffc451fdbULL, 0x995c4b23e1d1160bULL, 0x2b29a342daaddc6aULL, 0x4d61e56a525d225aULL,
+    0x43c952aaf5758e46ULL, 0x0000000000000000ULL, 0x2923370d7ac10983ULL, 0xaa858902220ea990ULL,
+    0x69a2e82f78565621ULL, 0x739372f4bf0b0fb8ULL, 0x780fd6fb82b37a31ULL, 0x02098986e0a466fdULL,
+    0x28609398374c18f1ULL, 0x29e73013be3651b9ULL, 0x461d798a66052b32ULL, 0xd659822019cc73beULL,
+    0xdbc3c57ead55b199ULL, 0xd60e073d896ed8d2ULL,
+};
+static constexpr unsigned int PM_ALWAYS_ROW0 = 0x000u;
+static constexpr unsigned int PM_ALWAYS_END4 = 0xfffu;
+static constexpr unsigned int PM_ALWAYS_END3 = 0x000u;
diff --git a/plonky2-aes_amd/csrc/prover_gpu.hip b/plonky2-aes_amd/csrc/prover_gpu.hip
--- a/plonky2-aes_amd/csrc/prover_gpu.hip
+++ b/plonky2-aes_amd/csrc/prover_gpu.hip
@@ -2291,6 +2291,17 @@
     HIPCHECK(hipMemcpy(states, d, count * 96, hipMemcpyDeviceToHost));
     return P2_OK;
 }
+int p2_gpu_merged_middle(uint64_t* states, size_t count, int device) {
+    if (count == 0 || count > (1u << 24)) return set_error("count out of range"), P2_ERR_INVALID;
+    if (int rc = pick_device(device)) return rc;
+    Allocs mem;
+    u64* d;
+    if (upload(mem, &d, (const u64*)states, count * 12)) return P2_ERR_HIP;
+    hipLaunchKernelGGL(k_merged_middle, g1(count, 256), dim3(256), 0, 0, d, count);
+    HIPCHECK(hipGetLastError());
+    HIPCHECK(hipMemcpy(states, d, count * 96, hipMemcpyDeviceToHost));
+    return P2_OK;
+}
 int p2_gpu_merkle_level(const uint64_t* child, size_t num_parents, size_t batch, uint64_t* parent, int device) {
     if (num_parents == 0 || batch == 0 || batch > 65535) return set_error("shape out of range"), P2_ERR_INVALID;
     if (int rc = pick_device(device)) return rc;
```
